# facebook/winterfell

Measured on NVIDIA H100. Metric: prover_ms, lower is better.
Workload: dtype u64

## Files before the change

include/winterfell_b200.h:

```cpp
#ifndef WINTERFELL_B200_H
#define WINTERFELL_B200_H

#include <stddef.h>
#include <stdint.h>

#ifdef __cplusplus
extern "C" {
#endif

#define WF_OK 0
#define WF_ERR_CUDA (-1)
#define WF_ERR_INVALID (-2)
#define WF_ERR_UNSUPPORTED (-3)
#define WF_ERR_STATE (-4)

#define WF_HASH_BLAKE3_256 0
#define WF_HASH_RP64_256 1
#define WF_HASH_RPJIVE64_256 2
#define WF_HASH_SHA3_256 4
#define WF_HASH_BLAKE3_192 3

typedef struct wf_ctx wf_ctx;
typedef struct wf_mat wf_mat;
typedef struct wf_tree wf_tree;
typedef struct wf_fri wf_fri;

int wf_ctx_create(wf_ctx** out, int device, void* stream);
void wf_ctx_destroy(wf_ctx* ctx);
const char* wf_last_error(const wf_ctx* ctx);
int wf_ctx_sync(wf_ctx* ctx);
uint64_t wf_ctx_launch_count(const wf_ctx* ctx);
int wf_ctx_mem_stats(const wf_ctx* ctx, uint64_t* live_buffers, uint64_t* live_bytes, uint64_t* pooled_bytes);
const char* wf_version(void);
int wf_ctx_set_profiling(wf_ctx* ctx, int on);
int wf_ctx_stage_times(wf_ctx* ctx, char* names, size_t names_cap, float* ms, size_t* count);

int wf_mat_from_host_columns(wf_ctx* ctx, const uint64_t* const* cols, uint32_t ncols, size_t nrows,
                             int ext_degree, int mont, wf_mat** out);
int wf_mat_from_device_columns(wf_ctx* ctx, const uint64_t* d_cols, uint32_t ncols, size_t nrows, wf_mat** out);
int wf_mat_select_columns(wf_ctx* ctx, const wf_mat* m, uint32_t first, uint32_t count, wf_mat** out);
int wf_mat_free(wf_ctx* ctx, wf_mat* m);
size_t wf_mat_rows(const wf_mat* m);
uint32_t wf_mat_cols(const wf_mat* m);
int wf_mat_to_columns(wf_ctx* ctx, const wf_mat* m, uint64_t* dst, int to_host, int mont);
int wf_mat_to_rows(wf_ctx* ctx, const wf_mat* m, uint64_t* dst, int to_host, int mont);
int wf_mat_read_rows(wf_ctx* ctx, const wf_mat* m, const uint64_t* positions, size_t k, uint64_t* dst, int mont);

int wf_mat_interpolate(wf_ctx* ctx, const wf_mat* evals, wf_mat** polys);
int wf_mat_evaluate(wf_ctx* ctx, const wf_mat* polys, wf_mat** evals);
int wf_mat_lde(wf_ctx* ctx, const wf_mat* polys, uint32_t log_blowup, wf_mat** lde);
int wf_mat_lde_into(wf_ctx* ctx, const wf_mat* polys, uint32_t log_blowup, wf_mat* lde);
int wf_mat_wrap_device(wf_ctx* ctx, uint64_t* d_segments, size_t rows, uint32_t cols, wf_mat** out);
int wf_trace_lde_from_host(wf_ctx* ctx, const uint64_t* const* cols, uint32_t ncols, size_t nrows, int mont, uint32_t log_blowup,
                           wf_mat** polys, wf_mat** lde);
int wf_mat_interpolate_with_offset(wf_ctx* ctx, const wf_mat* evals, uint64_t domain_offset, wf_mat** polys);

int wf_commit_rows(wf_ctx* ctx, int hash_id, const wf_mat* m, wf_tree** out);
int wf_commit_rows_partitioned(wf_ctx* ctx, int hash_id, const wf_mat* m, uint32_t partition_size, wf_tree** out);
int wf_tree_from_leaves(wf_ctx* ctx, int hash_id, const uint8_t* leaves, size_t nleaves, int leaves_on_device,
                        wf_tree** out);
int wf_tree_free(wf_ctx* ctx, wf_tree* t);
int wf_tree_root(wf_ctx* ctx, const wf_tree* t, uint8_t root[32]);
size_t wf_tree_num_leaves(const wf_tree* t);
int wf_tree_to_host(wf_ctx* ctx, const wf_tree* t, uint8_t* leaves, uint8_t* nodes);
int wf_tree_open_many(wf_ctx* ctx, const wf_tree* t, const uint64_t* positions, size_t k, uint8_t* leaves_out,
                      uint8_t* proof, size_t* proof_len);

typedef void (*wf_fri_commit_fn)(void* user, const uint8_t root[32]);
typedef void (*wf_fri_draw_fn)(void* user, uint64_t* alpha_out);
int wf_fri_build_layers(wf_ctx* ctx, int hash_id, const wf_mat* evals, int ext_degree, uint32_t folding_factor,
                        uint32_t remainder_max_degree, uint32_t blowup, wf_fri_commit_fn commit,
                        wf_fri_draw_fn draw_alpha, void* user, wf_fri** out);
int wf_fri_build_layers_default_channel(wf_ctx* ctx, int hash_id, const wf_mat* evals, int ext_degree,
                                        uint32_t folding_factor, uint32_t remainder_max_degree, uint32_t blowup,
                                        uint8_t* roots_out, size_t roots_cap, wf_fri** out);
uint32_t wf_fri_num_layers(const wf_fri* f);
size_t wf_fri_remainder(const wf_fri* f, uint64_t* coeffs, size_t cap_words);
int wf_fri_build_proof(wf_ctx* ctx, wf_fri* f, const uint64_t* positions, size_t k, uint8_t* out, size_t* len);
int wf_fri_free(wf_ctx* ctx, wf_fri* f);

int wf_prove_fib(wf_ctx* ctx, const uint64_t* const* trace_cols, int mont, uint32_t k, uint32_t log_n,
                 const uint64_t* results, const uint32_t* opts, uint8_t* proof, size_t* proof_len);

int wf_prove_air(wf_ctx* ctx, const uint64_t* air_desc, size_t air_desc_len, const uint64_t* const* trace_cols, int mont,
                 uint32_t log_n, const uint32_t* opts, uint8_t* proof, size_t* proof_len);

typedef int (*wf_aux_builder_fn)(void* user, const uint64_t* rand_elements, uint64_t* aux_out);
int wf_prove_air_aux(wf_ctx* ctx, const uint64_t* air_desc, size_t air_desc_len, const uint64_t* const* trace_cols, int mont,
                     uint32_t log_n, const uint32_t* opts, wf_aux_builder_fn aux_builder, void* aux_user, uint8_t* proof,
                     size_t* proof_len);

typedef int (*wf_aux_assertions_fn)(void* user, const uint64_t* rand_elements, uint64_t* values);
int wf_prove_air_aux_dyn(wf_ctx* ctx, const uint64_t* air_desc, size_t air_desc_len, const uint64_t* const* trace_cols, int mont,
                         uint32_t log_n, const uint32_t* opts, wf_aux_builder_fn aux_builder, wf_aux_assertions_fn aux_assertions,
                         void* aux_user, uint8_t* proof, size_t* proof_len);

int wf_prove_fib_dev(wf_ctx* ctx, const uint64_t* d_trace, uint32_t k, uint32_t log_n, const uint64_t* results,
                     const uint32_t* opts, uint8_t* proof, size_t* proof_len);

int wf_aux_build_check(const uint64_t* air_desc, size_t air_desc_len, const uint64_t* aux_build, size_t aux_build_len, uint32_t log_n,
                       char* msg, size_t msg_cap);
int wf_aux_build(wf_ctx* ctx, const uint64_t* air_desc, size_t air_desc_len, const uint64_t* aux_build, size_t aux_build_len,
                 const wf_mat* main_evals, const uint64_t* rand, uint32_t ext, wf_mat** aux);
int wf_prove_air_aux_built(wf_ctx* ctx, const uint64_t* air_desc, size_t air_desc_len, const uint64_t* aux_build, size_t aux_build_len,
                           const uint64_t* const* trace_cols, const uint64_t* d_trace, int mont, uint32_t log_n, const uint32_t* opts,
                           wf_aux_assertions_fn aux_assertions, void* aux_user, uint8_t* proof, size_t* proof_len);

int wf_prove_air_batch(wf_ctx* ctx, uint32_t batch, const uint64_t* const* air_descs, const size_t* air_desc_lens,
                       const uint64_t* aux_build, size_t aux_build_len, const uint64_t* const* trace_cols, const uint64_t* d_traces,
                       int mont, uint32_t log_n, const uint32_t* opts, uint8_t* const* proofs, size_t* proof_lens);
int wf_air_batch_check(uint32_t batch, const uint64_t* const* air_descs, const size_t* air_desc_lens, uint32_t log_n, uint32_t blowup,
                       char* msg, size_t msg_cap);

#define WF_VERIFY_ACCEPT               0
#define WF_VERIFY_MALFORMED            1
#define WF_VERIFY_OOD                  2
#define WF_VERIFY_POW                  3
#define WF_VERIFY_TRACE_QUERY          4
#define WF_VERIFY_CONSTRAINT_QUERY     5
#define WF_VERIFY_FRI_LAYER            6
#define WF_VERIFY_FRI_FOLD             7
#define WF_VERIFY_FRI_REMAINDER        8
#define WF_VERIFY_CONTEXT              9
#define WF_VERIFY_UNACCEPTABLE_OPTIONS 10
typedef int (*wf_aux_assertions_batch_fn)(void* user, uint32_t proof, const uint64_t* rand_elements, uint64_t* values);
int wf_verify_air_batch(wf_ctx* ctx, uint32_t batch, const uint64_t* const* air_descs, const size_t* air_desc_lens,
                        const uint8_t* const* proofs, const size_t* proof_lens, int hash_id,
                        const uint32_t* acceptable_opts, uint32_t num_acceptable,
                        wf_aux_assertions_batch_fn aux_assertions, void* aux_user, uint32_t* verdicts);

#define WF_VALID 0
#define WF_VIOLATION_MAIN_ASSERTION 1
#define WF_VIOLATION_AUX_ASSERTION 2
#define WF_VIOLATION_MAIN_TRANSITION 3
#define WF_VIOLATION_AUX_TRANSITION 4
#define WF_VIOLATION_DEGREES 5
#define WF_VIOLATION_CE_DOMAIN 6
typedef struct wf_validation {
    uint32_t kind;
    uint32_t index;
    uint64_t step;
    uint32_t column;
    uint32_t num_transition_constraints;
} wf_validation;
int wf_trace_validate(wf_ctx* ctx, const uint64_t* air_desc, size_t air_desc_len, const uint64_t* aux_build, size_t aux_build_len,
                      const uint64_t* const* aux_cols, const uint64_t* const* trace_cols, const uint64_t* d_trace, int mont,
                      const uint64_t* rand, uint32_t log_n, uint32_t ext, int check_degrees, wf_validation* report,
                      uint64_t* first_failing_step, uint64_t* expected_degrees, uint64_t* actual_degrees, char* msg, size_t msg_cap);
int wf_ctx_set_validation(wf_ctx* ctx, int on);

int wf_eval_constraints(wf_ctx* ctx, const uint64_t* air_desc, size_t air_desc_len, uint32_t log_n, uint32_t blowup, uint32_t ext,
                        const wf_mat* main_lde, const wf_mat* aux_lde, const uint64_t* coeffs, const uint64_t* aux_rand,
                        wf_mat** out);
int wf_composition_commit(wf_ctx* ctx, int hash_id, const wf_mat* comp_trace, uint32_t log_n, uint32_t blowup, uint32_t ext,
                          uint32_t num_cols, wf_mat** polys, wf_mat** lde, wf_tree** tree);
int wf_composition_commit_partitioned(wf_ctx* ctx, int hash_id, const wf_mat* comp_trace, uint32_t log_n, uint32_t blowup,
                                      uint32_t ext, uint32_t num_cols, uint32_t partition_size, wf_mat** polys, wf_mat** lde,
                                      wf_tree** tree);
int wf_mat_evaluate_at(wf_ctx* ctx, const wf_mat* polys, uint32_t ext, uint32_t col_ext, const uint64_t* z0, const uint64_t* z1,
                       uint64_t* out0, uint64_t* out1);
int wf_deep_compose(wf_ctx* ctx, uint32_t ext, const wf_mat* main_lde, const wf_mat* aux_lde, const wf_mat* cons_lde, uint32_t log_n,
                    const uint64_t* z, const uint64_t* coeffs, const uint64_t* ood_cur, const uint64_t* ood_next, wf_mat** out);
int wf_deep_compose_polys(wf_ctx* ctx, uint32_t ext, const wf_mat* main_polys, const wf_mat* aux_polys, const wf_mat* cons_polys,
                          uint32_t log_blowup, const uint64_t* z, const uint64_t* coeffs, wf_mat** out);

int wf_grind(wf_ctx* ctx, int hash_id, const uint8_t seed[32], uint32_t grinding, uint64_t* nonce);

typedef struct wf_comm {
    void* user;
    int rank, world;
    int (*exchange)(void* user, size_t nsend, const int* send_peer, const void* const* send, size_t nrecv,
                    const int* recv_peer, void* const* recv, size_t bytes);
    int (*all_gather_host)(void* user, const void* send, void* recv, size_t bytes);
    int (*all_reduce_sum)(void* user, void* d_buf, size_t words);
    int (*fork)(void* user);
    int (*join)(void* user);
} wf_comm;
int wf_shard_columns(uint32_t width, uint32_t world, uint32_t rank, uint32_t* first, uint32_t* count);
int wf_prove_fib_sharded(wf_ctx* ctx, const wf_comm* comm, const uint64_t* const* local_cols, const uint64_t* d_local, int mont,
                         uint32_t k, uint32_t log_n, const uint64_t* results, const uint32_t* opts, uint8_t* proof,
                         size_t* proof_len, double* stats);
int wf_prove_air_sharded(wf_ctx* ctx, const wf_comm* comm, const uint64_t* air_desc, size_t air_desc_len, const uint64_t* aux_build,
                         size_t aux_build_len, wf_aux_assertions_fn aux_assertions, void* aux_user, const uint64_t* const* local_cols,
                         const uint64_t* d_local, uint32_t local_count, int mont, uint32_t log_n, const uint32_t* opts, uint8_t* proof,
                         size_t* proof_len, double* stats);
int wf_trace_validate_sharded(wf_ctx* ctx, const wf_comm* comm, const uint64_t* air_desc, size_t air_desc_len,
                              const uint64_t* aux_build, size_t aux_build_len, const uint64_t* const* aux_cols,
                              const uint64_t* const* local_cols, const uint64_t* d_local, uint32_t local_count, int mont,
                              const uint64_t* rand, uint32_t log_n, uint32_t ext, int check_degrees, wf_validation* report,
                              uint64_t* first_failing_step, uint64_t* expected_degrees, uint64_t* actual_degrees,
                              char* msg, size_t msg_cap);

int wf_ctx_set_jit(wf_ctx* ctx, int on);
int wf_ctx_jit_stats(wf_ctx* ctx, uint64_t* compiled, uint64_t* cache_hits, uint64_t* fallbacks);
int wf_jit_compile_air(const uint64_t* air_desc, size_t air_desc_len, uint32_t ext, size_t* cubin_bytes, char* log, size_t log_cap);
int wf_air_check(const uint64_t* air_desc, size_t air_desc_len, uint32_t log_n, uint32_t blowup, char* msg, size_t msg_cap);

int wf_ntt_dev(wf_ctx* ctx, uint64_t* d_data, uint32_t log_n, uint32_t cols, int inverse);
int wf_hash_rows_dev(wf_ctx* ctx, int hash_id, const uint64_t* d_rows, size_t nrows, uint32_t cols, uint8_t* d_digests);
int wf_merkle_dev(wf_ctx* ctx, int hash_id, const uint8_t* d_leaves, size_t nleaves, uint8_t* d_nodes);
int wf_fri_fold_dev(wf_ctx* ctx, const uint64_t* d_evals, size_t len, int ext_degree, uint32_t folding_factor,
                    const uint64_t* alpha, uint64_t* d_next);

// ... 39 lines not shown
```

winterfell_b200/__init__.py:

```python
import ctypes as C
import os

import numpy as np

_HERE = os.path.dirname(os.path.abspath(__file__))
LIB_PATH = os.environ.get("WF_LIB_PATH") or os.path.join(_HERE, "libwinterfell_b200.so")

P = 0xFFFFFFFF00000001
HASH_BLAKE3_256 = 0
HASH_RP64_256 = 1
HASH_RPJIVE64_256 = 2
HASH_BLAKE3_192 = 3
HASH_SHA3_256 = 4

WF_OK = 0

u64p = C.POINTER(C.c_uint64)
u8p = C.POINTER(C.c_uint8)
vp = C.c_void_p

FRI_COMMIT_FN = C.CFUNCTYPE(None, C.c_void_p, u8p)
FRI_DRAW_FN = C.CFUNCTYPE(None, C.c_void_p, u64p)
AUX_BUILDER = C.CFUNCTYPE(C.c_int, C.c_void_p, u64p, u64p)
AUX_ASSERTIONS_BATCH = C.CFUNCTYPE(C.c_int, C.c_void_p, C.c_uint32, u64p, u64p)

VERIFY_ACCEPT, VERIFY_MALFORMED, VERIFY_OOD, VERIFY_POW, VERIFY_TRACE_QUERY, VERIFY_CONSTRAINT_QUERY, VERIFY_FRI_LAYER, \
    VERIFY_FRI_FOLD, VERIFY_FRI_REMAINDER, VERIFY_CONTEXT, VERIFY_UNACCEPTABLE_OPTIONS = range(11)

VALID, VIOLATION_MAIN_ASSERTION, VIOLATION_AUX_ASSERTION, VIOLATION_MAIN_TRANSITION, VIOLATION_AUX_TRANSITION, VIOLATION_DEGREES, \
    VIOLATION_CE_DOMAIN = range(7)


class Validation(C.Structure):
    _fields_ = [("kind", C.c_uint32), ("index", C.c_uint32), ("step", C.c_uint64), ("column", C.c_uint32),
                ("num_transition_constraints", C.c_uint32)]


def validation_dict(rep, first, exp, act, msg, check_degrees):
    k = rep.num_transition_constraints
    return {"kind": rep.kind, "index": rep.index, "step": rep.step, "column": rep.column,
            "first_failing_step": [None if int(v) == 2**64 - 1 else int(v) for v in first[:k]],
            "expected_degrees": [int(v) for v in exp[:k]] if check_degrees else None,
            "actual_degrees": [int(v) for v in act[:k]] if check_degrees else None,
            "msg": msg.value.decode(errors="replace")}


_lib = None

_SIGS = [
    ("wf_ctx_create", C.c_int, [C.POINTER(vp), C.c_int, vp]),
    ("wf_ctx_destroy", None, [vp]),
    ("wf_last_error", C.c_char_p, [vp]),
    ("wf_ctx_sync", C.c_int, [vp]),
    ("wf_ctx_launch_count", C.c_uint64, [vp]),
    ("wf_ctx_mem_stats", C.c_int, [vp, C.POINTER(C.c_uint64), C.POINTER(C.c_uint64), C.POINTER(C.c_uint64)]),
    ("wf_version", C.c_char_p, []),
    ("wf_ctx_set_profiling", C.c_int, [vp, C.c_int]),
    ("wf_ctx_stage_times", C.c_int, [vp, C.c_char_p, C.c_size_t, C.POINTER(C.c_float), C.POINTER(C.c_size_t)]),
    ("wf_mat_from_host_columns", C.c_int, [vp, C.POINTER(u64p), C.c_uint32, C.c_size_t, C.c_int, C.c_int, C.POINTER(vp)]),
    ("wf_mat_from_device_columns", C.c_int, [vp, vp, C.c_uint32, C.c_size_t, C.POINTER(vp)]),
    ("wf_mat_select_columns", C.c_int, [vp, vp, C.c_uint32, C.c_uint32, C.POINTER(vp)]),
    ("wf_mat_free", C.c_int, [vp, vp]),
    ("wf_mat_rows", C.c_size_t, [vp]),
    ("wf_mat_cols", C.c_uint32, [vp]),
    ("wf_mat_to_columns", C.c_int, [vp, vp, vp, C.c_int, C.c_int]),
    ("wf_mat_to_rows", C.c_int, [vp, vp, vp, C.c_int, C.c_int]),
    ("wf_mat_read_rows", C.c_int, [vp, vp, u64p, C.c_size_t, u64p, C.c_int]),
    ("wf_mat_interpolate", C.c_int, [vp, vp, C.POINTER(vp)]),
    ("wf_mat_evaluate", C.c_int, [vp, vp, C.POINTER(vp)]),
    ("wf_mat_lde", C.c_int, [vp, vp, C.c_uint32, C.POINTER(vp)]),
    ("wf_mat_lde_into", C.c_int, [vp, vp, C.c_uint32, vp]),
    ("wf_mat_wrap_device", C.c_int, [vp, vp, C.c_size_t, C.c_uint32, C.POINTER(vp)]),
    ("wf_trace_lde_from_host", C.c_int, [vp, C.POINTER(u64p), C.c_uint32, C.c_size_t, C.c_int, C.c_uint32, C.POINTER(vp), C.POINTER(vp)]),
    ("wf_mat_interpolate_with_offset", C.c_int, [vp, vp, C.c_uint64, C.POINTER(vp)]),
    ("wf_commit_rows", C.c_int, [vp, C.c_int, vp, C.POINTER(vp)]),
    ("wf_commit_rows_partitioned", C.c_int, [vp, C.c_int, vp, C.c_uint32, C.POINTER(vp)]),
    ("wf_tree_from_leaves", C.c_int, [vp, C.c_int, vp, C.c_size_t, C.c_int, C.POINTER(vp)]),
    ("wf_tree_free", C.c_int, [vp, vp]),
    ("wf_tree_root", C.c_int, [vp, vp, u8p]),
    ("wf_tree_num_leaves", C.c_size_t, [vp]),
    ("wf_tree_to_host", C.c_int, [vp, vp, u8p, u8p]),
    ("wf_tree_open_many", C.c_int, [vp, vp, u64p, C.c_size_t, u8p, u8p, C.POINTER(C.c_size_t)]),
    ("wf_fri_build_layers", C.c_int, [vp, C.c_int, vp, C.c_int, C.c_uint32, C.c_uint32, C.c_uint32, FRI_COMMIT_FN, FRI_DRAW_FN, vp, C.POINTER(vp)]),
    ("wf_fri_build_layers_default_channel", C.c_int, [vp, C.c_int, vp, C.c_int, C.c_uint32, C.c_uint32, C.c_uint32, u8p, C.c_size_t, C.POINTER(vp)]),
    ("wf_fri_num_layers", C.c_uint32, [vp]),
    ("wf_fri_remainder", C.c_size_t, [vp, u64p, C.c_size_t]),
    ("wf_fri_build_proof", C.c_int, [vp, vp, u64p, C.c_size_t, u8p, C.POINTER(C.c_size_t)]),
    ("wf_fri_free", C.c_int, [vp, vp]),
    ("wf_prove_fib", C.c_int, [vp, C.POINTER(u64p), C.c_int, C.c_uint32, C.c_uint32, u64p, C.POINTER(C.c_uint32), u8p, C.POINTER(C.c_size_t)]),
    ("wf_prove_air", C.c_int, [vp, u64p, C.c_size_t, C.POINTER(u64p), C.c_int, C.c_uint32, C.POINTER(C.c_uint32), u8p, C.POINTER(C.c_size_t)]),
    ("wf_prove_air_aux", C.c_int, [vp, u64p, C.c_size_t, C.POINTER(u64p), C.c_int, C.c_uint32, C.POINTER(C.c_uint32), AUX_BUILDER, vp,
                                   u8p, C.POINTER(C.c_size_t)]),
        ("wf_prove_air_aux_dyn", C.c_int, [vp, u64p, C.c_size_t, C.POINTER(u64p), C.c_int, C.c_uint32, C.POINTER(C.c_uint32), AUX_BUILDER, AUX_BUILDER, vp,
                                   u8p, C.POINTER(C.c_size_t)]),
    ("wf_aux_build_check", C.c_int, [u64p, C.c_size_t, u64p, C.c_size_t, C.c_uint32, C.c_char_p, C.c_size_t]),
    ("wf_aux_build", C.c_int, [vp, u64p, C.c_size_t, u64p, C.c_size_t, vp, u64p, C.c_uint32, C.POINTER(vp)]),
    ("wf_prove_air_aux_built", C.c_int, [vp, u64p, C.c_size_t, u64p, C.c_size_t, C.POINTER(u64p), vp, C.c_int, C.c_uint32,
                                         C.POINTER(C.c_uint32), AUX_BUILDER, vp, u8p, C.POINTER(C.c_size_t)]),
    ("wf_eval_constraints", C.c_int, [vp, u64p, C.c_size_t, C.c_uint32, C.c_uint32, C.c_uint32, vp, vp, u64p, u64p, C.POINTER(vp)]),
    ("wf_composition_commit", C.c_int, [vp, C.c_int, vp, C.c_uint32, C.c_uint32, C.c_uint32, C.c_uint32, C.POINTER(vp), C.POINTER(vp), C.POINTER(vp)]),
    ("wf_composition_commit_partitioned", C.c_int, [vp, C.c_int, vp, C.c_uint32, C.c_uint32, C.c_uint32, C.c_uint32, C.c_uint32, C.POINTER(vp),
                                                    C.POINTER(vp), C.POINTER(vp)]),
    ("wf_mat_evaluate_at", C.c_int, [vp, vp, C.c_uint32, C.c_uint32, u64p, u64p, u64p, u64p]),
    ("wf_deep_compose", C.c_int, [vp, C.c_uint32, vp, vp, vp, C.c_uint32, u64p, u64p, u64p, u64p, C.POINTER(vp)]),
    ("wf_deep_compose_polys", C.c_int, [vp, C.c_uint32, vp, vp, vp, C.c_uint32, u64p, u64p, C.POINTER(vp)]),
    ("wf_prove_fib_dev", C.c_int, [vp, vp, C.c_uint32, C.c_uint32, u64p, C.POINTER(C.c_uint32), u8p, C.POINTER(C.c_size_t)]),
    ("wf_grind", C.c_int, [vp, C.c_int, u8p, C.c_uint32, C.POINTER(C.c_uint64)]),
    ("wf_ntt_dev", C.c_int, [vp, vp, C.c_uint32, C.c_uint32, C.c_int]),
    ("wf_hash_rows_dev", C.c_int, [vp, C.c_int, vp, C.c_size_t, C.c_uint32, vp]),
    ("wf_merkle_dev", C.c_int, [vp, C.c_int, vp, C.c_size_t, vp]),
    ("wf_fri_fold_dev", C.c_int, [vp, vp, C.c_size_t, C.c_int, C.c_uint32, u64p, vp]),
    ("wf_field_ops_dev", C.c_int, [vp, vp, vp, C.c_size_t, vp]),
    ("wf_field_shifts_dev", C.c_int, [vp, vp, C.c_size_t, vp]),
    ("wf_rescue_ops_dev", C.c_int, [vp, vp, vp, C.c_size_t, vp]),
    ("wf_rescue_permute_dev", C.c_int, [vp, C.c_int, vp, vp, C.c_size_t, vp]),
    ("wf_ext_ops_dev", C.c_int, [vp, C.c_uint32, vp, vp, C.c_size_t, vp]),
    ("wf_acc_ops_dev", C.c_int, [vp, vp, vp, C.c_uint32, C.c_size_t, vp]),
    ("wf_eval_constraints_window", C.c_int, [vp, u64p, C.c_size_t, C.c_uint32, C.c_uint32, C.c_uint32, vp, vp, u64p, u64p, C.c_size_t,
                                             C.c_size_t, C.POINTER(vp)]),
    ("wf_eval_constraints_fib", C.c_int, [vp, C.c_uint32, u64p, C.c_uint32, C.c_uint32, C.c_uint32, vp, u64p, C.c_size_t, C.c_size_t,
                                          C.POINTER(vp)]),
    ("wf_eval_constraints_subcoset", C.c_int, [vp, u64p, C.c_size_t, C.c_uint32, C.c_uint32, C.c_uint32, vp, vp, u64p, u64p, C.c_size_t,
                                               C.POINTER(vp)]),
    ("wf_eval_constraints_fib_subcoset", C.c_int, [vp, C.c_uint32, u64p, C.c_uint32, C.c_uint32, C.c_uint32, vp, u64p, C.c_size_t,
                                                   C.POINTER(vp)]),
    ("wf_ctx_set_jit", C.c_int, [vp, C.c_int]),
    ("wf_ctx_jit_stats", C.c_int, [vp, C.POINTER(C.c_uint64), C.POINTER(C.c_uint64), C.POINTER(C.c_uint64)]),
    ("wf_jit_compile_air", C.c_int, [u64p, C.c_size_t, C.c_uint32, C.POINTER(C.c_size_t), C.c_char_p, C.c_size_t]),
    ("wf_air_check", C.c_int, [u64p, C.c_size_t, C.c_uint32, C.c_uint32, C.c_char_p, C.c_size_t]),
    ("wf_prove_air_batch", C.c_int, [vp, C.c_uint32, C.POINTER(u64p), C.POINTER(C.c_size_t), u64p, C.c_size_t, C.POINTER(u64p), vp, C.c_int,
                                     C.c_uint32, C.POINTER(C.c_uint32), C.POINTER(u8p), C.POINTER(C.c_size_t)]),
    ("wf_trace_validate", C.c_int, [vp, u64p, C.c_size_t, u64p, C.c_size_t, C.POINTER(u64p), C.POINTER(u64p), vp, C.c_int, u64p, C.c_uint32,
                                    C.c_uint32, C.c_int, C.POINTER(Validation), u64p, u64p, u64p, C.c_char_p, C.c_size_t]),
    ("wf_ctx_set_validation", C.c_int, [vp, C.c_int]),
    ("wf_air_batch_check", C.c_int, [C.c_uint32, C.POINTER(u64p), C.POINTER(C.c_size_t), C.c_uint32, C.c_uint32, C.c_char_p, C.c_size_t]),
    ("wf_verify_air_batch", C.c_int, [vp, C.c_uint32, C.POINTER(u64p), C.POINTER(C.c_size_t), C.POINTER(u8p), C.POINTER(C.c_size_t), C.c_int,
                                      C.POINTER(C.c_uint32), C.c_uint32, AUX_ASSERTIONS_BATCH, vp, C.POINTER(C.c_uint32)]),
    ("wf_host_hash_elements", C.c_int, [C.c_int, u64p, C.c_size_t, u8p]),
    ("wf_host_merge", C.c_int, [C.c_int, u8p, u8p]),
    ("wf_host_merge_with_int", C.c_int, [C.c_int, u8p, C.c_uint64, u8p]),
    ("wf_host_mul", C.c_uint64, [C.c_uint64, C.c_uint64]),
    ("wf_host_mul_2exp", C.c_uint64, [C.c_uint64, C.c_uint32]),
    ("wf_host_mont_to_canonical", C.c_uint64, [C.c_uint64]),
    ("wf_host_canonical_to_mont", C.c_uint64, [C.c_uint64]),
    ("wf_host_write_usize", C.c_size_t, [C.c_uint64, u8p]),
    ("wf_host_coin_draw", C.c_int, [C.c_int, u64p, C.c_size_t, u8p, C.c_int, C.c_size_t, u64p]),
    ("wf_host_build_fib_trace", C.c_int, [C.c_uint32, C.c_size_t, u64p, u64p]),
    ("wf_host_sharded_opening_plan", C.c_long, [C.c_size_t, C.c_int, C.c_int, u64p, C.c_size_t, u64p, u64p, C.c_size_t]),
    ("wf_prove_fib_sharded", C.c_int, [vp, vp, C.POINTER(u64p), vp, C.c_int, C.c_uint32, C.c_uint32, u64p, C.POINTER(C.c_uint32), u8p,
                                       C.POINTER(C.c_size_t), C.POINTER(C.c_double)]),
    ("wf_shard_columns", C.c_int, [C.c_uint32, C.c_uint32, C.c_uint32, C.POINTER(C.c_uint32), C.POINTER(C.c_uint32)]),
    ("wf_prove_air_sharded", C.c_int, [vp, vp, u64p, C.c_size_t, u64p, C.c_size_t, AUX_BUILDER, vp, C.POINTER(u64p), vp, C.c_uint32,
                                       C.c_int, C.c_uint32, C.POINTER(C.c_uint32), u8p, C.POINTER(C.c_size_t), C.POINTER(C.c_double)]),
    ("wf_trace_validate_sharded", C.c_int, [vp, vp, u64p, C.c_size_t, u64p, C.c_size_t, C.POINTER(u64p), C.POINTER(u64p), vp, C.c_uint32,
                                            C.c_int, u64p, C.c_uint32, C.c_uint32, C.c_int, C.POINTER(Validation), u64p, u64p, u64p,
                                            C.c_char_p, C.c_size_t]),
]


def declared_symbols():
    return [s[0] for s in _SIGS]


def lib():
    global _lib
    if _lib is None:
        if not os.path.exists(LIB_PATH):
            raise RuntimeError(
                f"{LIB_PATH} is missing: build it with winterfell_b200/build.sh "
                "(python -c 'import __graft_entry__ as g; g.build()'). There is no CPU fallback.")
        L = C.CDLL(LIB_PATH)
        for name, res, args in _SIGS:
            fn = getattr(L, name)
            fn.restype = res
            fn.argtypes = args
        _lib = L
    return _lib


class WfError(RuntimeError):
    pass


def _u64(a):
    a = np.ascontiguousarray(a, dtype=np.uint64)
    return a, a.ctypes.data_as(u64p)


def _u8(a):
    a = np.ascontiguousarray(a, dtype=np.uint8)
    return a, a.ctypes.data_as(u8p)


class Context:

    def __init__(self, device=0, stream=0):
        self.L = lib()
        h = vp()
        r = self.L.wf_ctx_create(C.byref(h), device, vp(stream))
        if r != WF_OK:
            raise WfError(f"wf_ctx_create failed ({r}): no usable CUDA device — this library has no CPU path")
        self.h = h

    def close(self):
        if getattr(self, "h", None):
            self.L.wf_ctx_destroy(self.h)
            self.h = None

    def __del__(self):
        try:
            self.close()
        except Exception:
            pass

    def check(self, r):
        if r != WF_OK:
            raise WfError(f"error {r}: {self.L.wf_last_error(self.h).decode()}")

    def sync(self):
        self.check(self.L.wf_ctx_sync(self.h))

    @property
    def launches(self):
        return self.L.wf_ctx_launch_count(self.h)
# ... 337 lines not shown
        ptrs, dev = None, None
        if isinstance(trace, int):
            if n is None:
                raise ValueError("n is required with a device trace pointer")
            dev = vp(trace)
        else:
            a = np.ascontiguousarray(trace, dtype=np.uint64)
            c, n = a.shape
            ptrs = (u64p * c)(*[a[j].ctypes.data_as(u64p) for j in range(c)])
        rp = aps = bp = None
        bl = 0
        if rand is not None:
            r_, rp = _u64(np.asarray(rand, dtype=np.uint64).reshape(-1))
        if aux is not None:
            x_ = np.ascontiguousarray(aux, dtype=np.uint64)
            aps = (u64p * x_.shape[0])(*[x_[j].ctypes.data_as(u64p) for j in range(x_.shape[0])])
        if aux_build is not None:
            b_, bp = _u64(aux_build)
            bl = b_.size
        cap = 1 + len(desc)
        first, exp, act = (np.zeros(cap, dtype=np.uint64) for _ in range(3))
        rep = Validation()
        msg = C.create_string_buffer(1 << 16)
        self.check(self.L.wf_trace_validate(self.h, dp, d_.size, bp, bl, aps, ptrs, dev, int(mont), rp, int(n).bit_length() - 1, ext,
                                            int(check_degrees), C.byref(rep), first.ctypes.data_as(u64p), exp.ctypes.data_as(u64p),
                                            act.ctypes.data_as(u64p), msg, 1 << 16))
        return validation_dict(rep, first, exp, act, msg, check_degrees)

    def set_validation(self, on):
        self.check(self.L.wf_ctx_set_validation(self.h, int(on)))

    def prove_fib_dev(self, d_trace, k, log_n, results, opts, out_buf=None):
        r_, rp = _u64(results)
        o_ = np.ascontiguousarray(opts, dtype=np.uint32)
        buf = out_buf if out_buf is not None else np.zeros(1 << 23, dtype=np.uint8)
        ln = C.c_size_t(buf.size)
        self.check(self.L.wf_prove_fib_dev(self.h, vp(d_trace), k, log_n, rp, o_.ctypes.data_as(C.POINTER(C.c_uint32)),
                                           buf.ctypes.data_as(u8p), C.byref(ln)))
        return buf[: ln.value].tobytes()

    def set_profiling(self, on):
        self.check(self.L.wf_ctx_set_profiling(self.h, int(on)))

    def stage_times(self):
        names = C.create_string_buffer(4096)
        ms = (C.c_float * 64)()
        cnt = C.c_size_t(64)
        self.check(self.L.wf_ctx_stage_times(self.h, names, 4096, ms, C.byref(cnt)))
        nm = [x for x in names.value.decode().split(",") if x]
        return [(nm[i], float(ms[i])) for i in range(cnt.value)]

    def grind(self, hash_id, seed: bytes, grinding):
        t_, tp = _u8(np.frombuffer(seed, dtype=np.uint8))
        nonce = C.c_uint64(0)
        self.check(self.L.wf_grind(self.h, hash_id, tp, grinding, C.byref(nonce)))
        return nonce.value

    def ntt_dev(self, dptr, log_n, cols, inverse=False):
        self.check(self.L.wf_ntt_dev(self.h, vp(dptr), log_n, cols, int(inverse)))

    def hash_rows_dev(self, hash_id, d_rows, nrows, cols, d_digests):
        self.check(self.L.wf_hash_rows_dev(self.h, hash_id, vp(d_rows), nrows, cols, vp(d_digests)))

    def merkle_dev(self, hash_id, d_leaves, nleaves, d_nodes):
        self.check(self.L.wf_merkle_dev(self.h, hash_id, vp(d_leaves), nleaves, vp(d_nodes)))

    def field_ops_dev(self, d_a, d_b, n, d_out):
        self.check(self.L.wf_field_ops_dev(self.h, vp(d_a), vp(d_b), n, vp(d_out)))

    def field_shifts_dev(self, d_a, n, d_out):
        self.check(self.L.wf_field_shifts_dev(self.h, vp(d_a), n, vp(d_out)))

    def rescue_ops_dev(self, d_a, d_b, n, d_out):
        self.check(self.L.wf_rescue_ops_dev(self.h, vp(d_a), vp(d_b), n, vp(d_out)))

    def rescue_permute_dev(self, hash_id, d_states, d_values, n, d_out):
        self.check(self.L.wf_rescue_permute_dev(self.h, hash_id, vp(d_states), vp(d_values), n, vp(d_out)))

    def set_jit(self, on):
        self.check(self.L.wf_ctx_set_jit(self.h, int(on)))

    def jit_stats(self):
        a, b, c = C.c_uint64(0), C.c_uint64(0), C.c_uint64(0)
        self.check(self.L.wf_ctx_jit_stats(self.h, C.byref(a), C.byref(b), C.byref(c)))
        return {"compiled": a.value, "cache_hits": b.value, "fallbacks": c.value}

    def ext_ops_dev(self, ext, d_a, d_b, n, d_out):
        self.check(self.L.wf_ext_ops_dev(self.h, ext, vp(d_a), vp(d_b), n, vp(d_out)))

    def acc_ops_dev(self, d_x, d_y, k, n, d_out):
        self.check(self.L.wf_acc_ops_dev(self.h, vp(d_x), vp(d_y), k, n, vp(d_out)))

    def fri_fold_dev(self, d_evals, length, ext_degree, folding, alpha, d_next):
        a_, ap = _u64(alpha)
        self.check(self.L.wf_fri_fold_dev(self.h, vp(d_evals), length, ext_degree, folding, ap, vp(d_next)))


class Mat:
    def __init__(self, ctx, h):
        self.ctx, self.h = ctx, h

    def free(self):
        if self.h:
            self.ctx.L.wf_mat_free(self.ctx.h, self.h)
            self.h = None

    @property
    def rows(self):
        return self.ctx.L.wf_mat_rows(self.h)

    @property
    def cols(self):
        return self.ctx.L.wf_mat_cols(self.h)

    def to_columns(self, mont=False):
        o = np.zeros((self.cols, self.rows), dtype=np.uint64)
        self.ctx.check(self.ctx.L.wf_mat_to_columns(self.ctx.h, self.h, vp(o.ctypes.data), 1, int(mont)))
        return o

    def to_rows(self, mont=False):
        o = np.zeros((self.rows, self.cols), dtype=np.uint64)
        self.ctx.check(self.ctx.L.wf_mat_to_rows(self.ctx.h, self.h, vp(o.ctypes.data), 1, int(mont)))
        return o

    def to_device_rows(self, dptr):
        self.ctx.check(self.ctx.L.wf_mat_to_rows(self.ctx.h, self.h, vp(dptr), 0, 0))

    def read_rows(self, positions, mont=False):
        p_, pp = _u64(positions)
        o = np.zeros((p_.size, self.cols), dtype=np.uint64)
        self.ctx.check(self.ctx.L.wf_mat_read_rows(self.ctx.h, self.h, pp, p_.size, o.ctypes.data_as(u64p), int(mont)))
        return o

    def _unary(self, fn, *extra):
        h = vp()
        self.ctx.check(fn(self.ctx.h, self.h, *extra, C.byref(h)))
        return Mat(self.ctx, h)

    def select_columns(self, first, count):
        return self._unary(self.ctx.L.wf_mat_select_columns, first, count)

    def interpolate(self):
        return self._unary(self.ctx.L.wf_mat_interpolate)

    def evaluate(self):
        return self._unary(self.ctx.L.wf_mat_evaluate)

    def lde_into(self, log_blowup, out):
        self.ctx.check(self.ctx.L.wf_mat_lde_into(self.ctx.h, self.h, log_blowup, out.h))

    def lde(self, log_blowup):
        return self._unary(self.ctx.L.wf_mat_lde, log_blowup)

    def interpolate_with_offset(self, offset):
        return self._unary(self.ctx.L.wf_mat_interpolate_with_offset, offset)


class Tree:
    def __init__(self, ctx, h):
        self.ctx, self.h = ctx, h

    def free(self):
        if self.h:
            self.ctx.L.wf_tree_free(self.ctx.h, self.h)
            self.h = None

    @property
    def num_leaves(self):
        return self.ctx.L.wf_tree_num_leaves(self.h)

    def root(self):
        o = np.zeros(32, dtype=np.uint8)
        self.ctx.check(self.ctx.L.wf_tree_root(self.ctx.h, self.h, o.ctypes.data_as(u8p)))
        return o.tobytes()

    def to_host(self):
        n = self.num_leaves
        lv = np.zeros((n, 32), dtype=np.uint8)
        nd = np.zeros((n, 32), dtype=np.uint8)
        self.ctx.check(self.ctx.L.wf_tree_to_host(self.ctx.h, self.h, lv.ctypes.data_as(u8p), nd.ctypes.data_as(u8p)))
        return lv, nd

    def open_many(self, positions):
        p_, pp = _u64(positions)
        k = p_.size
        lv = np.zeros((k, 32), dtype=np.uint8)
        cap = 64 + k * 40 * 33
        buf = np.zeros(cap, dtype=np.uint8)
        ln = C.c_size_t(cap)
        self.ctx.check(self.ctx.L.wf_tree_open_many(self.ctx.h, self.h, pp, k, lv.ctypes.data_as(u8p),
                                                    buf.ctypes.data_as(u8p), C.byref(ln)))
        return lv, buf[: ln.value].tobytes()


class Fri:
    def __init__(self, ctx, h, d):
        self.ctx, self.h, self.d = ctx, h, d

    def free(self):
        if self.h:
            self.ctx.L.wf_fri_free(self.ctx.h, self.h)
            self.h = None

    @property
    def num_layers(self):
        return self.ctx.L.wf_fri_num_layers(self.h)

    def remainder(self):
        buf = np.zeros(4096, dtype=np.uint64)
        n = self.ctx.L.wf_fri_remainder(self.h, buf.ctypes.data_as(u64p), buf.size)
        return buf[: n * self.d].copy()

    def build_proof(self, positions):
        p_, pp = _u64(positions)
        cap = 1 << 22
        buf = np.zeros(cap, dtype=np.uint8)
        ln = C.c_size_t(cap)
        self.ctx.check(self.ctx.L.wf_fri_build_proof(self.ctx.h, self.h, pp, p_.size, buf.ctypes.data_as(u8p), C.byref(ln)))
        return buf[: ln.value].tobytes()


def build_fib_trace(k, n, out=None):
    tr = out if out is not None else np.empty((2 * k, n), dtype=np.uint64)
    assert tr.shape == (2 * k, n) and tr.dtype == np.uint64 and tr.flags["C_CONTIGUOUS"]
    res = np.zeros(k, dtype=np.uint64)
    if lib().wf_host_build_fib_trace(k, n, tr.ctypes.data_as(u64p), res.ctypes.data_as(u64p)) != WF_OK:
        raise WfError("wf_host_build_fib_trace: bad arguments")
    return tr, res


def sharded_opening_plan(n_global, world, rank, positions):
    p_, pp = _u64(positions)
    cap = 64 * max(len(p_), 1) * 64
    want, idx = np.zeros(cap, dtype=np.uint64), np.zeros(cap, dtype=np.uint64)
    cnt = lib().wf_host_sharded_opening_plan(n_global, world, rank, pp, len(p_), want.ctypes.data_as(u64p), idx.ctypes.data_as(u64p), cap)
    if cnt < 0:
        raise WfError("wf_host_sharded_opening_plan: bad arguments")
    return want[:cnt].copy(), idx[:cnt].copy()


def host_hash_elements(hash_id, elems):
    e_, ep = _u64(np.asarray(elems, dtype=np.uint64).reshape(-1))
    o = np.zeros(32, dtype=np.uint8)
    lib().wf_host_hash_elements(hash_id, ep, e_.size, o.ctypes.data_as(u8p))
    return o.tobytes()


def host_merge(hash_id, a, b):
    t_, tp = _u8(np.frombuffer(a + b, dtype=np.uint8))
    o = np.zeros(32, dtype=np.uint8)
    lib().wf_host_merge(hash_id, tp, o.ctypes.data_as(u8p))
    return o.tobytes()


def host_merge_with_int(hash_id, seed, value):
    t_, tp = _u8(np.frombuffer(seed, dtype=np.uint8))
    o = np.zeros(32, dtype=np.uint8)
    lib().wf_host_merge_with_int(hash_id, tp, value, o.ctypes.data_as(u8p))
    return o.tobytes()


def air_check(desc, log_n, blowup):
    d_, dp = _u64(desc)
    msg = C.create_string_buffer(512)
    rc = lib().wf_air_check(dp, d_.size, log_n, blowup, msg, 512)
    return rc, msg.value.decode(errors="replace")


def _aux_value_count(desc):
    d = [int(x) for x in desc]
    p = 1
    def skip_degrees(p):
        cnt = d[p]; p += 1
        for _ in range(cnt):
            p += 2 + d[p + 1]
        return p
    p = skip_degrees(p)
    cnt = d[p]; p += 1
    for _ in range(cnt):
        p += 1 + d[p]
    p += 1 + d[p]
    p += 1
    p += 1 + 4 * d[p]
    cnt = d[p]; p += 1
    for _ in range(cnt):
        p += 4 + d[p + 3]
    p += 1 + d[p]
    p += 1
    if p == len(d):
        return 0
    p += 2
    p = skip_degrees(p)
    p += 1
    p += 1 + 4 * d[p]
    cnt = d[p]; p += 1
    total = 0
    for _ in range(cnt):
        total += d[p + 3]
        p += 4 + 3 * d[p + 3]
    return total


def air_batch_check(descs, log_n, blowup):
    ds = [np.ascontiguousarray(d, dtype=np.uint64) for d in descs]
    dps = (u64p * len(ds))(*[d.ctypes.data_as(u64p) for d in ds])
    dls = (C.c_size_t * len(ds))(*[d.size for d in ds])
# ... 20 lines not shown
```

winterfell_b200/csrc/capi.cu:

```cuda
#include <cuda_runtime.h>
#include <stdarg.h>
#include <stdio.h>

#include <algorithm>
#include <map>
#include <set>
#include <string>
#include <thread>
#include <utility>
#include <vector>

#include "internal.hpp"
#include "alg_hash.cuh"

void wf_mark(wf_ctx* ctx, const char* name) {
    if (!ctx->profiling) return;
    cudaEvent_t e;
    if (cudaEventCreate(&e) != cudaSuccess) return;
    cudaEventRecord(e, ctx->st);
    ctx->marks.push_back({name, e});
}
int wf_fail(wf_ctx* ctx, int code, const char* fmt, ...) {
    char buf[512];
    va_list ap;
// ... 146 lines not shown
        u64 sk = gl_mul(GL_GENERATOR, gl_pow(g, k));
        bases[k] = logR == 0 ? sk : gl_pow(sk, C);
    }
    LdeTables t{nullptr, nullptr};
    void *p, *pb;
    CK(cudaMalloc(&p, b * cnt * 8));
    CK(cudaMalloc(&pb, b * 8));
    CK(cudaMemcpyAsync(pb, bases.data(), b * 8, cudaMemcpyHostToDevice, ctx->st));
    pow_table2_kernel<<<(unsigned)((b * cnt + 255) / 256), 256, 0, ctx->st>>>((u64*)p, (u64*)pb, cnt, b);
    ctx->launches++;
    CK(cudaGetLastError());
    CK(cudaStreamSynchronize(ctx->st));
    cudaFree(pb);
    t.pre = (u64*)p;
    if (logR != 0) {
        void* q;
        CK(cudaMalloc(&q, C * 8));
        pow_table_kernel<<<(unsigned)((C + 255) / 256), 256, 0, ctx->st>>>((u64*)q, GL_GENERATOR, 1, C);
        ctx->launches++;
        CK(cudaGetLastError());
        t.pow7 = (u64*)q;
    }
    ctx->lde_tabs[key] = t;
    *out = t;
    return WF_OK;
}

static void pass_defaults(NttPassParams& p, const SegMatrix& in, const SegMatrix& out) {
    memset(&p, 0, sizeof(p));
    p.in = in.base;
    p.out = out.base;
    p.in_seg_stride = in.seg_stride;
    p.out_seg_stride = out.seg_stride;
    p.W = in.W;
    p.out_W = (u32)out.W;
    p.out_row_mul = 1;
    p.cconst = 1;
}
static int split3(wf_ctx* ctx, u32 log_n, u32* lr, u32* lc, u32* lr2, u32* lc2) {
    *lr = (log_n + 2) / 3;
    *lc = log_n - *lr;
    split_log(*lc, lr2, lc2);
    if (*lr2 == 0 || *lc2 > NTT_MAX_LOGS || *lr > NTT_MAX_LOGS)
        return wf_fail(ctx, WF_ERR_UNSUPPORTED, "transform of 2^%u points exceeds the three-pass limit", log_n);
    return WF_OK;
}

static int run_ntt(wf_ctx* ctx, const SegMatrix& in, SegMatrix& out, const SegMatrix* tmp, u32 log_n, int inverse) {
    u32 logR, logC;
    split_log(log_n, &logR, &logC);
    u64 inv_n = gl_inv(((u64)1 << log_n) % GL_P);
    NttPassParams p;
    if (logC > NTT_MAX_LOGS) {
        if (!tmp) return wf_fail(ctx, WF_ERR_STATE, "run_ntt: scratch matrix required");
        u32 lr, lc, lr2, lc2;
        CKI(split3(ctx, log_n, &lr, &lc, &lr2, &lc2));
        pass_defaults(p, in, *tmp);
        p.logS = (int)lr; p.logR = lr; p.logC = lc; p.inverse = inverse;
        p.has_post = 1; p.logM = log_n; p.a_mul = 1; p.b_mul = 0; p.cconst = inverse ? inv_n : 1;
        CKI(launch_pass(ctx, NTT_STRIDED, p, in.nseg(), 1));
        pass_defaults(p, *tmp, *tmp);
        p.in_batch_stride = p.out_batch_stride = ((size_t)1 << lc) * in.W;
        p.logS = (int)lr2; p.logR = lr2; p.logC = lc2; p.inverse = inverse;
        p.has_post = 1; p.logM = lc; p.a_mul = 1; p.b_mul = 0;
        CKI(launch_pass(ctx, NTT_STRIDED, p, in.nseg(), 1u << lr));
        pass_defaults(p, *tmp, out);
        p.in_batch_stride = ((size_t)1 << lc) * in.W;
        p.logS = (int)lc2; p.logR = lr2; p.logC = lc2; p.inverse = inverse;
        p.out_row_mul = 1u << lr; p.out_row_add = 1;
        CKI(launch_pass(ctx, NTT_CONTIG, p, in.nseg(), 1u << lr));
        return WF_OK;
    }
    if (logR == 0) {
        pass_defaults(p, in, out);
        p.logS = (int)logC; p.logR = 0; p.logC = logC; p.inverse = inverse;
        if (inverse) p.cconst = inv_n;
        return launch_pass(ctx, NTT_CONTIG, p, in.nseg(), 1);
    }
    if (!tmp) return wf_fail(ctx, WF_ERR_STATE, "run_ntt: scratch matrix required");
    pass_defaults(p, in, *tmp);
    p.logS = (int)logR; p.logR = logR; p.logC = logC; p.inverse = inverse;
    p.has_post = 1; p.logM = log_n; p.a_mul = 1; p.b_mul = 0; p.cconst = inverse ? inv_n : 1;
    CKI(launch_pass(ctx, NTT_STRIDED, p, in.nseg(), 1));
    pass_defaults(p, *tmp, out);
    p.logS = (int)logC; p.logR = logR; p.logC = logC; p.inverse = inverse;
    return launch_pass(ctx, NTT_CONTIG, p, in.nseg(), 1);
}

static int run_lde(wf_ctx* ctx, const SegMatrix& polys, SegMatrix& out, u32 log_n, u32 log_b, u32 out_col0 = 0, u32 k0 = 0, u32 k1 = 0,
                   u32 row_mul = 0, u32 row_add = 1) {
    u32 logR, logC;
    split_log(log_n, &logR, &logC);
    u32 b = 1u << log_b;
    if (k1 == 0) k1 = b;
    if (row_mul == 0) { row_mul = b; row_add = 1; }
    LdeTables tabs;
    NttPassParams p;
    if (logC > NTT_MAX_LOGS) {
        u32 lr, lc, lr2, lc2;
        CKI(split3(ctx, log_n, &lr, &lc, &lr2, &lc2));
        CKI(get_lde_tables(ctx, log_n, log_b, lr, &tabs));
        SegMatrix y = polys;
        void* yp;
        CKI(wf_dev_alloc(ctx, polys.words() * 8, &yp));
        y.base = (u64*)yp;
        int rc = WF_OK;
        for (u32 k = k0; k < k1 && rc == WF_OK; k++) {
            pass_defaults(p, polys, y);
            p.logS = (int)lr; p.logR = lr; p.logC = lc;
            p.pre_tab = tabs.pre + ((size_t)k << lr); p.pre_batch_stride = 0;
            p.has_post = 1; p.logM = log_n + log_b; p.a_mul = b; p.b_mul = 1; p.batch0 = k;
            p.ctab = tabs.pow7;
            rc = launch_pass(ctx, NTT_STRIDED, p, polys.nseg(), 1);
            if (rc != WF_OK) break;
            pass_defaults(p, y, y);
            p.in_batch_stride = p.out_batch_stride = ((size_t)1 << lc) * polys.W;
            p.logS = (int)lr2; p.logR = lr2; p.logC = lc2;
            p.has_post = 1; p.logM = lc; p.a_mul = 1; p.b_mul = 0;
            rc = launch_pass(ctx, NTT_STRIDED, p, polys.nseg(), 1u << lr);
            if (rc != WF_OK) break;
            pass_defaults(p, y, out);
            p.in_batch_stride = ((size_t)1 << lc) * polys.W;
            p.logS = (int)lc2; p.logR = lr2; p.logC = lc2;
            p.out_row_mul = row_mul << lr; p.out_row_add = row_mul; p.out_col0 = out_col0;
            p.out = out.base + (size_t)(k - k0) * row_add * out.W;
            rc = launch_pass(ctx, NTT_CONTIG, p, polys.nseg(), 1u << lr);
        }
        wf_dev_free(ctx, yp);
        return rc;
    }
    CKI(get_lde_tables(ctx, log_n, log_b, logR, &tabs));
    if (logR == 0) {
        pass_defaults(p, polys, out);
        p.logS = (int)logC; p.logR = 0; p.logC = logC;
        p.pre_tab = tabs.pre + ((size_t)k0 << log_n); p.pre_batch_stride = (size_t)1 << log_n;
        p.out_row_mul = row_mul; p.out_row_add = row_add; p.out_col0 = out_col0;
        return launch_pass(ctx, NTT_CONTIG, p, polys.nseg(), k1 - k0);
    }
    pass_defaults(p, polys, out);
    p.logS = (int)logR; p.logR = logR; p.logC = logC;
    p.pre_tab = tabs.pre + ((size_t)k0 << logR); p.pre_batch_stride = (size_t)1 << logR;
    p.has_post = 1; p.logM = log_n + log_b; p.a_mul = b; p.b_mul = 1; p.batch0 = k0;
    p.ctab = tabs.pow7;
    p.y_in_out = 1; p.out_row_mul = row_mul; p.out_row_add = row_add; p.out_col0 = out_col0;
    CKI(launch_pass(ctx, NTT_STRIDED, p, polys.nseg(), k1 - k0));
    pass_defaults(p, polys, out);
    p.in = out.base;
    p.in_seg_stride = out.seg_stride;
    p.logS = (int)logC; p.logR = logR; p.logC = logC;
    p.y_in_out = 1; p.out_row_mul = row_mul; p.out_row_add = row_add; p.out_col0 = out_col0;
    return launch_pass(ctx, NTT_CONTIG, p, polys.nseg(), k1 - k0);
}

template <int K>
__device__ __forceinline__ void field_shift_store(u64 a, u64* out, size_t n, size_t i, int slot) { out[(4 + slot) * n + i] = gl_mul_2exp<K>(a); }
__global__ void field_ops_kernel(const u64* a, const u64* b, size_t n, u64* out) {
    size_t i = (size_t)blockIdx.x * blockDim.x + threadIdx.x;
    if (i >= n) return;
    u64 x = a[i], y = b[i];
    out[i] = gl_mul(x, y);
    out[n + i] = gl_add(x, y);
    out[2 * n + i] = gl_sub(x, y);
    out[3 * n + i] = x ? gl_inv(x) : 0;
    u64 s = x, d = y;
    gl_butterfly(s, d);
    if (s != out[n + i] || d != out[2 * n + i]) out[n + i] = ~0ULL;
    field_shift_store<1>(x, out, n, i, 0);   field_shift_store<3>(x, out, n, i, 1);   field_shift_store<6>(x, out, n, i, 2);
    field_shift_store<12>(x, out, n, i, 3);  field_shift_store<24>(x, out, n, i, 4);  field_shift_store<31>(x, out, n, i, 5);
    field_shift_store<32>(x, out, n, i, 6);  field_shift_store<33>(x, out, n, i, 7);  field_shift_store<48>(x, out, n, i, 8);
    field_shift_store<63>(x, out, n, i, 9);  field_shift_store<64>(x, out, n, i, 10); field_shift_store<65>(x, out, n, i, 11);
    field_shift_store<72>(x, out, n, i, 12); field_shift_store<80>(x, out, n, i, 13); field_shift_store<84>(x, out, n, i, 14);
    field_shift_store<90>(x, out, n, i, 15); field_shift_store<95>(x, out, n, i, 16); field_shift_store<96>(x, out, n, i, 17);
}
template <int... K>
__device__ __forceinline__ void field_shifts_all(u64 x, u64* out, size_t n, size_t i, std::integer_sequence<int, K...>) {
    ((out[(size_t)K * n + i] = gl_mul_2exp<K>(x)), ...);
}
__global__ void field_shifts_kernel(const u64* a, size_t n, u64* out) {
    size_t i = (size_t)blockIdx.x * blockDim.x + threadIdx.x;
    if (i >= n) return;
    field_shifts_all(a[i], out, n, i, std::make_integer_sequence<int, 97>{});
}

__global__ void rescue_weak_kernel(const u64* a, const u64* b, size_t n, u64* out) {
    size_t i = (size_t)blockIdx.x * blockDim.x + threadIdx.x;
    if (i >= n) return;
    out[i] = gl_mul_weak(a[i], b[i]);
    out[n + i] = gl_sqr_weak(a[i]);
    out[2 * n + i] = rp64_exp7(a[i]);
}
template <int G>
__global__ void rescue_inv7_kernel(const u64* a, size_t n, u64* out) {
    size_t t = (size_t)blockIdx.x * blockDim.x + threadIdx.x;
    if (t >= n / G) return;
    u64 s[G];
#pragma unroll
    for (int e = 0; e < G; e++) s[e] = a[t * G + e];
    rp64_inv7_group<G>(s);
#pragma unroll
    for (int e = 0; e < G; e++) out[t * G + e] = s[e];
}
__global__ void rescue_mds_kernel(const u64* a, size_t n, u64* out12, u64* out8) {
    size_t t = (size_t)blockIdx.x * blockDim.x + threadIdx.x;
    if (t < n / 12) {
        u64 s[12];
        for (int e = 0; e < 12; e++) s[e] = a[t * 12 + e];
        rp64_mds(s);
        for (int e = 0; e < 12; e++) out12[t * 12 + e] = s[e];
    }
    if (t < n / 8) {
        u64 s[8];
        for (int e = 0; e < 8; e++) s[e] = a[t * 8 + e];
        rpj_mds(s);
        for (int e = 0; e < 8; e++) out8[t * 8 + e] = s[e];
    }
}
template <int HASH, int W>
__global__ void rescue_permute_kernel(const u64* in, const u64* values, size_t n, u64* out) {
    size_t i = (size_t)blockIdx.x * blockDim.x + threadIdx.x;
    if (i >= n) return;
    u64 s[W];
#pragma unroll
    for (int e = 0; e < W; e++) s[e] = in[i * W + e];
    u64 m[4], mi[4];
    alg_merge<HASH>(s, m);
    alg_merge_with_int<HASH>(s, values[i], mi);
    if (HASH == WF_HASH_RP64_256) rp64_permute(s);
    else rpj_permute(s);
#pragma unroll
    for (int e = 0; e < W; e++) out[i * W + e] = s[e];
#pragma unroll
    for (int e = 0; e < 4; e++) { out[n * W + i * 4 + e] = m[e]; out[n * (W + 4) + i * 4 + e] = mi[e]; }
}

template <int D>
__global__ void ext_ops_kernel(const u64* a, const u64* b, size_t n, u64* out) {
    size_t i = (size_t)blockIdx.x * blockDim.x + threadIdx.x;
    if (i >= n) return;
    GlExt<D> x, y;
#pragma unroll
    for (int q = 0; q < D; q++) { x.v[q] = a[i * D + q]; y.v[q] = b[i * D + q]; }
    const GlExt<D> r[6] = {ext_mul(x, y), ext_inv(x), ext_frobenius(x), ext_mul_base(x, y.v[0]), ext_add(x, y), ext_sub(x, y)};
#pragma unroll
    for (int k = 0; k < 6; k++)
#pragma unroll
        for (int q = 0; q < D; q++) out[((size_t)k * n + i) * D + q] = r[k].v[q];
}

__global__ void acc_ops_kernel(const u64* x, const u64* y, u32 k, size_t n, u64* out) {
    size_t i = (size_t)blockIdx.x * blockDim.x + threadIdx.x;
    if (i >= n) return;
    GlAcc a = acc_zero();
    for (u32 j = 0; j < k; j++) acc_mad(a, x[i * k + j], y[i * k + j]);
    u64* o = out + i * 6;
    o[0] = a.w0; o[1] = a.w1; o[2] = a.w2; o[3] = a.w3; o[4] = a.w4;
    o[5] = acc_reduce(a);
}

template <int K>
static u64 m2e(u64 x) { return gl_mul_2exp<K>(x); }

extern "C" {

const char* wf_version(void) { return "winterfell_b200 0.1 (sm_90a)"; }

int wf_ctx_create(wf_ctx** out, int device, void* stream) {
    if (!out) return WF_ERR_INVALID;
    *out = nullptr;
    int n = 0;
    cudaError_t e = cudaGetDeviceCount(&n);
    if (e != cudaSuccess || n == 0) return WF_ERR_CUDA;
    if (device < 0 || device >= n) return WF_ERR_INVALID;
    if (cudaSetDevice(device) != cudaSuccess) return WF_ERR_CUDA;
    wf_ctx* ctx = new wf_ctx();
    ctx->device = device;
    ctx->st = (cudaStream_t)stream;
    ctx->launches = 0;
    ctx->pinned = nullptr;
    ctx->pinned_bytes = 0;
    ctx->profiling = false;
    *out = ctx;
    return WF_OK;
}
void wf_ctx_destroy(wf_ctx* ctx) {
    if (!ctx) return;
    cudaSetDevice(ctx->device);
    cudaStreamSynchronize(ctx->st);
    for (auto& kv : ctx->pool) cudaFree(kv.second);
    for (auto& kv : ctx->live) cudaFree(kv.first);
    for (auto& kv : ctx->tw) cudaFree(kv.second);
    for (auto& kv : ctx->lde_tabs) { cudaFree(kv.second.pre); if (kv.second.pow7) cudaFree(kv.second.pow7); }
    if (ctx->pinned) cudaFreeHost(ctx->pinned);
    for (auto& kv : ctx->ipc_opened) cudaIpcCloseMemHandle(kv.second);
    for (auto& kv : ctx->jit_cache) if (kv.second.first) cudaLibraryUnload((cudaLibrary_t)kv.second.first);
    for (int i = 0; i < 4; i++) if (ctx->push_st[i]) { cudaStreamSynchronize(ctx->push_st[i]); cudaStreamDestroy(ctx->push_st[i]); }
    for (int i = 0; i < 16; i++) if (ctx->push_ev[i]) cudaEventDestroy(ctx->push_ev[i]);
    if (ctx->copy_st) {
        cudaStreamSynchronize(ctx->copy_st);
        for (int i = 0; i < 2; i++) { cudaEventDestroy(ctx->ev_up[i]); cudaEventDestroy(ctx->ev_used[i]); }
        cudaEventDestroy(ctx->ev_start);
        cudaStreamDestroy(ctx->copy_st);
    }
    delete ctx;
}
int wf_ctx_set_profiling(wf_ctx* ctx, int on) {
    if (!ctx) return WF_ERR_INVALID;
    ctx->profiling = on != 0;
    for (auto& m : ctx->marks) cudaEventDestroy(m.second);
    ctx->marks.clear();
    return WF_OK;
}
int wf_ctx_stage_times(wf_ctx* ctx, char* names, size_t names_cap, float* ms, size_t* count) {
    if (!ctx || !names || !ms || !count) return WF_ERR_INVALID;
    CK(cudaStreamSynchronize(ctx->st));
    size_t n = ctx->marks.size() > 0 ? ctx->marks.size() - 1 : 0, used = 0;
    if (n > *count) n = *count;
    names[0] = 0;
    for (size_t i = 0; i < n; i++) {
        CK(cudaEventElapsedTime(&ms[i], ctx->marks[i].second, ctx->marks[i + 1].second));
        const std::string& nm = ctx->marks[i + 1].first;
        if (used + nm.size() + 2 < names_cap) { memcpy(names + used, nm.c_str(), nm.size()); used += nm.size(); names[used++] = ','; names[used] = 0; }
    }
    *count = n;
    for (auto& m : ctx->marks) cudaEventDestroy(m.second);
    ctx->marks.clear();
    return WF_OK;
}
const char* wf_last_error(const wf_ctx* ctx) { return ctx ? ctx->err.c_str() : "no context (is a CUDA device present?)"; }
int wf_ctx_sync(wf_ctx* ctx) { wf_use_device(ctx); CK(cudaStreamSynchronize(ctx->st)); return WF_OK; }
uint64_t wf_ctx_launch_count(const wf_ctx* ctx) { return ctx->launches; }
int wf_ctx_mem_stats(const wf_ctx* ctx, uint64_t* live_buffers, uint64_t* live_bytes, uint64_t* pooled_bytes) {
    if (!ctx) return WF_ERR_INVALID;
    uint64_t lb = 0, pb = 0;
    for (auto& kv : ctx->live) lb += kv.second;
    for (auto& kv : ctx->pool) pb += kv.first;
    if (live_buffers) *live_buffers = ctx->live.size();
    if (live_bytes) *live_bytes = lb;
    if (pooled_bytes) *pooled_bytes = pb;
    return WF_OK;
}

int wf_mat_from_device_columns(wf_ctx* ctx, const uint64_t* d_cols, uint32_t ncols, size_t nrows, wf_mat** out) {
    if (!ctx || !d_cols || !out || ncols == 0 || nrows == 0) return wf_fail(ctx, WF_ERR_INVALID, "bad arguments");
    wf_mat* m;
    CKI(wf_mat_alloc(ctx, nrows, ncols, &m));
    CK(layout_cols_to_seg(d_cols, nrows, 1, 0, m->m, ctx->st));
    ctx->launches++;
    *out = m;
    return WF_OK;
}

int wf_mat_from_host_columns(wf_ctx* ctx, const uint64_t* const* cols, uint32_t ncols, size_t nrows, int ext_degree,
                             int mont, wf_mat** out) {
    if (!ctx || !cols || !out || ncols == 0 || nrows == 0 || ext_degree < 1 || ext_degree > 3)
        return wf_fail(ctx, WF_ERR_INVALID, "bad arguments");
    size_t col_words = nrows * ext_degree;
    void* stage;
    CKI(wf_dev_alloc(ctx, (size_t)ncols * col_words * 8, &stage));
    for (uint32_t j = 0; j < ncols; j++)
        CK(cudaMemcpyAsync((u64*)stage + (size_t)j * col_words, cols[j], col_words * 8, cudaMemcpyHostToDevice, ctx->st));
    wf_mat* m;
    int r = wf_mat_alloc(ctx, nrows, ncols * ext_degree, &m);
    if (r != WF_OK) { wf_dev_free(ctx, stage); return r; }
    CK(layout_cols_to_seg((u64*)stage, nrows, ext_degree, mont, m->m, ctx->st));
    ctx->launches++;
    wf_dev_free(ctx, stage);
    *out = m;
    return WF_OK;
}
int wf_mat_wrap_device(wf_ctx* ctx, uint64_t* d_segments, size_t rows, uint32_t cols, wf_mat** out) {
    if (!ctx || !d_segments || !out || rows == 0 || cols == 0) return wf_fail(ctx, WF_ERR_INVALID, "bad arguments");
    wf_mat* m = new wf_mat();
    m->m.rows = rows;
    m->m.cols = cols;
    m->m.W = seg_width_for(cols);
    m->m.seg_stride = rows * m->m.W;
    m->m.base = d_segments;
    *out = m;
    return WF_OK;
}
int wf_mat_select_columns(wf_ctx* ctx, const wf_mat* m, uint32_t first, uint32_t count, wf_mat** out) {
    if (!ctx || !m || !out || count == 0 || first + count > m->m.cols) return wf_fail(ctx, WF_ERR_INVALID, "bad column range");
    wf_mat* o;
    CKI(wf_mat_alloc(ctx, m->m.rows, count, &o));
    CK(layout_select_cols(m->m, first, o->m, ctx->st));
    ctx->launches++;
    *out = o;
    return WF_OK;
}
int wf_mat_free(wf_ctx* ctx, wf_mat* m) {
    if (!m) return WF_OK;
    wf_dev_free(ctx, m->m.base);
    delete m;
    return WF_OK;
}
size_t wf_mat_rows(const wf_mat* m) { return m->m.rows; }
uint32_t wf_mat_cols(const wf_mat* m) { return m->m.cols; }

static int mat_export(wf_ctx* ctx, const wf_mat* m, uint64_t* dst, int to_host, int mont, int row_major) {
    if (!ctx || !m || !dst) return wf_fail(ctx, WF_ERR_INVALID, "bad arguments");
    size_t words = m->m.rows * m->m.cols;
    u64* d = dst;
    void* tmp = nullptr;
    if (to_host) { CKI(wf_dev_alloc(ctx, words * 8, &tmp)); d = (u64*)tmp; }
    CK(layout_seg_to_flat(m->m, d, row_major, mont, ctx->st));
    ctx->launches++;
    if (to_host) {
        CK(cudaMemcpyAsync(dst, d, words * 8, cudaMemcpyDeviceToHost, ctx->st));
        CK(cudaStreamSynchronize(ctx->st));
        wf_dev_free(ctx, tmp);
    }
    return WF_OK;
}
int wf_mat_to_columns(wf_ctx* ctx, const wf_mat* m, uint64_t* dst, int to_host, int mont) { return mat_export(ctx, m, dst, to_host, mont, 0); }
int wf_mat_to_rows(wf_ctx* ctx, const wf_mat* m, uint64_t* dst, int to_host, int mont) { return mat_export(ctx, m, dst, to_host, mont, 1); }

int wf_mat_read_rows(wf_ctx* ctx, const wf_mat* m, const uint64_t* positions, size_t k, uint64_t* dst, int mont) {
    if (!ctx || !m || !positions || !dst) return wf_fail(ctx, WF_ERR_INVALID, "bad arguments");
    if (k == 0) return WF_OK;
    for (size_t i = 0; i < k; i++)
        if (positions[i] >= m->m.rows) return wf_fail(ctx, WF_ERR_INVALID, "row %llu out of range", (unsigned long long)positions[i]);
    void *dpos, *dout;
    CKI(wf_dev_alloc(ctx, k * 8, &dpos));
    CKI(wf_dev_alloc(ctx, k * m->m.cols * 8, &dout));
    CK(cudaMemcpyAsync(dpos, positions, k * 8, cudaMemcpyHostToDevice, ctx->st));
    CK(layout_gather_rows(m->m, (const u64*)dpos, k, (u64*)dout, mont, ctx->st));
    ctx->launches++;
    CK(cudaMemcpyAsync(dst, dout, k * m->m.cols * 8, cudaMemcpyDeviceToHost, ctx->st));
    CK(cudaStreamSynchronize(ctx->st));
    wf_dev_free(ctx, dpos);
    wf_dev_free(ctx, dout);
    return WF_OK;
}

static int log2_exact(size_t n, u32* out) {
    if (n == 0 || (n & (n - 1))) return -1;
    u32 l = 0;
    while (((size_t)1 << l) < n) l++;
    *out = l;
    return 0;
}

static int mat_transform(wf_ctx* ctx, const wf_mat* in, int inverse, wf_mat** out) {
    if (!ctx || !in || !out) return wf_fail(ctx, WF_ERR_INVALID, "bad arguments");
    u32 log_n;
    if (log2_exact(in->m.rows, &log_n) || log_n < 1) return wf_fail(ctx, WF_ERR_INVALID, "rows must be a power of two >= 2");
    wf_mat* o;
    CKI(wf_mat_alloc_w(ctx, in->m.rows, in->m.cols, in->m.W, &o));
    SegMatrix tmp = in->m;
    void* tp = nullptr;
    if (log_n > NTT_MAX_LOGS) {
        int r = wf_dev_alloc(ctx, in->m.words() * 8, &tp);
        if (r != WF_OK) { wf_mat_free(ctx, o); return r; }
        tmp.base = (u64*)tp;
    }
    int r = run_ntt(ctx, in->m, o->m, tp ? &tmp : nullptr, log_n, inverse);
    wf_dev_free(ctx, tp);
    if (r != WF_OK) { wf_mat_free(ctx, o); return r; }
    *out = o;
    return WF_OK;
}
int wf_mat_interpolate(wf_ctx* ctx, const wf_mat* evals, wf_mat** polys) { return mat_transform(ctx, evals, 1, polys); }
int wf_mat_evaluate(wf_ctx* ctx, const wf_mat* polys, wf_mat** evals) { return mat_transform(ctx, polys, 0, evals); }

int wf_mat_lde(wf_ctx* ctx, const wf_mat* polys, uint32_t log_blowup, wf_mat** lde) {
    if (!ctx || !polys || !lde) return wf_fail(ctx, WF_ERR_INVALID, "bad arguments");
    u32 log_n;
    if (log2_exact(polys->m.rows, &log_n) || log_n < 1) return wf_fail(ctx, WF_ERR_INVALID, "rows must be a power of two >= 2");
    if (log_blowup > 7 || log_n + log_blowup > 32) return wf_fail(ctx, WF_ERR_INVALID, "bad blowup");
    wf_mat* o;
    CKI(wf_mat_alloc(ctx, polys->m.rows << log_blowup, polys->m.cols, &o));
    int r = run_lde(ctx, polys->m, o->m, log_n, log_blowup);
    if (r != WF_OK) { wf_mat_free(ctx, o); return r; }
    *lde = o;
    return WF_OK;
}

int wf_mat_lde_into(wf_ctx* ctx, const wf_mat* polys, uint32_t log_blowup, wf_mat* lde) {
    if (!ctx || !polys || !lde) return wf_fail(ctx, WF_ERR_INVALID, "bad arguments");
    u32 log_n;
    if (log2_exact(polys->m.rows, &log_n) || log_n < 1) return wf_fail(ctx, WF_ERR_INVALID, "rows must be a power of two >= 2");
    if (log_blowup > 7 || lde->m.rows != (polys->m.rows << log_blowup) || lde->m.cols != polys->m.cols || lde->m.W != polys->m.W)
        return wf_fail(ctx, WF_ERR_INVALID, "output matrix does not match the LDE shape");
    return run_lde(ctx, polys->m, lde->m, log_n, log_blowup);
}

int wf_mat_lde_cosets(wf_ctx* ctx, const wf_mat* polys, uint32_t log_blowup, uint32_t k0, uint32_t k1, wf_mat* lde) {
    if (!ctx || !polys || !lde) return wf_fail(ctx, WF_ERR_INVALID, "bad arguments");
    u32 log_n;
    if (log2_exact(polys->m.rows, &log_n) || log_n < 1) return wf_fail(ctx, WF_ERR_INVALID, "rows must be a power of two >= 2");
    if (log_blowup > 7 || k0 >= k1 || k1 > (1u << log_blowup) || lde->m.rows != polys->m.rows * (k1 - k0) || lde->m.cols != polys->m.cols ||
        lde->m.W != polys->m.W || ((k1 - k0) & (k1 - k0 - 1)))
        return wf_fail(ctx, WF_ERR_INVALID, "coset range / output matrix do not match");
    return run_lde(ctx, polys->m, lde->m, log_n, log_blowup, 0, k0, k1, 1, (u32)polys->m.rows);
}

int wf_mat_lde_from_coset(wf_ctx* ctx, const wf_mat* polys, uint32_t log_blowup, uint32_t k0, wf_mat* lde) {
    if (!ctx || !polys || !lde) return wf_fail(ctx, WF_ERR_INVALID, "bad arguments");
    u32 log_n;
    if (log2_exact(polys->m.rows, &log_n) || log_n < 1) return wf_fail(ctx, WF_ERR_INVALID, "rows must be a power of two >= 2");
    if (log_blowup > 7 || k0 >= (1u << log_blowup) || lde->m.rows != (polys->m.rows << log_blowup) || lde->m.cols != polys->m.cols ||
        lde->m.W != polys->m.W)
        return wf_fail(ctx, WF_ERR_INVALID, "coset / output matrix do not match the LDE shape");
    SegMatrix view = lde->m;
    view.base += (size_t)k0 * view.W;
    return run_lde(ctx, polys->m, view, log_n, log_blowup, 0, k0, 1u << log_blowup);
}

int wf_trace_lde_from_host(wf_ctx* ctx, const uint64_t* const* cols, uint32_t ncols, size_t nrows, int mont, uint32_t log_blowup,
                           wf_mat** polys_out, wf_mat** lde_out) {
    return wf_trace_lde_cosetwise(ctx, cols, nullptr, ncols, nrows, mont, log_blowup, polys_out, lde_out, false, nullptr);
}
int wf_trace_lde_cosetwise(wf_ctx* ctx, const uint64_t* const* cols, const uint64_t* d_cols, uint32_t ncols, size_t nrows, int mont,
                           uint32_t log_blowup, wf_mat** polys_out, wf_mat** lde_out, bool coset_major,
                           const std::function<int(u32)>* after_coset) {
    if (!ctx || (!cols && !d_cols) || !polys_out || !lde_out || ncols == 0) return wf_fail(ctx, WF_ERR_INVALID, "bad arguments");
    u32 log_n;
    if (log2_exact(nrows, &log_n) || log_n < 1) return wf_fail(ctx, WF_ERR_INVALID, "rows must be a power of two >= 2");
    if (log_blowup > 7 || log_n + log_blowup > 32) return wf_fail(ctx, WF_ERR_INVALID, "bad blowup");
    if (coset_major && (!*lde_out || (*lde_out)->m.rows != (nrows << log_blowup) || (*lde_out)->m.W < seg_width_for(ncols) ||
                        (*lde_out)->m.cols != ncols))
        return wf_fail(ctx, WF_ERR_INVALID, "coset-major output must be preallocated");
    const int Wout = coset_major ? (*lde_out)->m.W : seg_width_for(ncols);
    const u32 nseg_out = (ncols + Wout - 1) / Wout;
    const u32 nb = 1u << log_blowup;
    auto extend = [&](const SegMatrix& pv, SegMatrix& ov, u32 out_col0, bool last) -> int {
        if (!after_coset || !last) {
            if (!coset_major) return run_lde(ctx, pv, ov, log_n, log_blowup, out_col0);
            return run_lde(ctx, pv, ov, log_n, log_blowup, out_col0, 0, nb, 1, (u32)nrows);
        }
        for (u32 k = 0; k < nb; k++) {
            SegMatrix ok = ov;
            ok.base += (coset_major ? (size_t)k * nrows : (size_t)k) * ov.W;
            if (coset_major) CKI(run_lde(ctx, pv, ok, log_n, log_blowup, out_col0, k, k + 1, 1, (u32)nrows));
            else CKI(run_lde(ctx, pv, ok, log_n, log_blowup, out_col0, k, k + 1, nb, 1));
            CKI((*after_coset)(k));
        }
        return WF_OK;
    };
    int Wc = nseg_out >= 2 ? Wout : (Wout >= 4 ? Wout / 2 : 0);
    if (d_cols || Wc == 0 || log_n < 12) {
        wf_mat* tr;
        if (d_cols) CKI(wf_mat_from_device_columns(ctx, d_cols, ncols, nrows, &tr));
        else CKI(wf_mat_from_host_columns(ctx, cols, ncols, nrows, 1, mont, &tr));
        int r = wf_mat_interpolate(ctx, tr, polys_out);
        wf_mat_free(ctx, tr);
        if (r != WF_OK) return r;
        if (!coset_major && !after_coset) return wf_mat_lde(ctx, *polys_out, log_blowup, lde_out);
        if (!coset_major) CKI(wf_mat_alloc(ctx, nrows << log_blowup, ncols, lde_out));
        const SegMatrix& pm = (*polys_out)->m;
        if (pm.W == Wout) return extend(pm, (*lde_out)->m, 0, true);
        for (u32 g = 0; g < pm.nseg(); g++) {
            SegMatrix pv = pm, ov = (*lde_out)->m;
            pv.base += (size_t)g * pm.seg_stride;
            pv.cols = std::min<u32>(pm.W, ncols - g * pm.W);
            ov.base += (size_t)(g * pm.W / Wout) * ov.seg_stride;
            ov.cols = pv.cols;
            CKI(extend(pv, ov, g * pm.W % Wout, g + 1 == pm.nseg()));
        }
        return WF_OK;
    }
    if (!ctx->copy_st) {
        CK(cudaStreamCreateWithFlags(&ctx->copy_st, cudaStreamNonBlocking));
        for (int i = 0; i < 2; i++) {
            CK(cudaEventCreateWithFlags(&ctx->ev_up[i], cudaEventDisableTiming));
            CK(cudaEventCreateWithFlags(&ctx->ev_used[i], cudaEventDisableTiming));
        }
        CK(cudaEventCreateWithFlags(&ctx->ev_start, cudaEventDisableTiming));
    }
    const u32 nchunks = (ncols + Wc - 1) / Wc;
    wf_mat *polys = nullptr, *lde = nullptr, *tr = nullptr;
    void* stage[2] = {nullptr, nullptr};
    void* tmp = nullptr;
    auto release = [&](bool results_too) {
        wf_mat_free(ctx, tr);
        for (int i = 0; i < 2; i++) wf_dev_free(ctx, stage[i]);
        wf_dev_free(ctx, tmp);
        if (results_too) { wf_mat_free(ctx, polys); if (!coset_major) wf_mat_free(ctx, lde); }
    };
    auto body = [&]() -> int {
        CKI(wf_mat_alloc_w(ctx, nrows, ncols, Wc, &polys));
        if (coset_major) lde = *lde_out;
        else CKI(wf_mat_alloc(ctx, nrows << log_blowup, ncols, &lde));
        CKI(wf_mat_alloc_w(ctx, nrows, Wc, Wc, &tr));
        for (int i = 0; i < 2; i++) CKI(wf_dev_alloc(ctx, (size_t)Wc * nrows * 8, &stage[i]));
        CKI(wf_dev_alloc(ctx, (size_t)Wc * nrows * 8, &tmp));
        if (lde->m.W > (int)ncols) CK(cudaMemsetAsync(lde->m.base, 0, lde->m.words() * 8, ctx->st));
        CK(cudaEventRecord(ctx->ev_start, ctx->st));
        CK(cudaStreamWaitEvent(ctx->copy_st, ctx->ev_start, 0));
        for (u32 k = 0; k < nchunks; k++) {
            const u32 c0 = k * Wc, cw = std::min<u32>(Wc, ncols - c0);
            const int sb = k & 1;
            if (k >= 2) CK(cudaStreamWaitEvent(ctx->copy_st, ctx->ev_used[sb], 0));
            for (u32 j = 0; j < cw; j++)
                CK(cudaMemcpyAsync((u64*)stage[sb] + (size_t)j * nrows, cols[c0 + j], nrows * 8, cudaMemcpyHostToDevice, ctx->copy_st));
            CK(cudaEventRecord(ctx->ev_up[sb], ctx->copy_st));
            CK(cudaStreamWaitEvent(ctx->st, ctx->ev_up[sb], 0));
            SegMatrix trv = tr->m;
            trv.cols = cw;
            CK(layout_cols_to_seg((const u64*)stage[sb], nrows, 1, mont, trv, ctx->st));
            CK(cudaEventRecord(ctx->ev_used[sb], ctx->st));
            ctx->launches++;
            SegMatrix pv = polys->m;
            pv.base = polys->m.base + (size_t)k * polys->m.seg_stride;
            pv.cols = cw;
            SegMatrix tv = trv;
            tv.base = (u64*)tmp;
            CKI(run_ntt(ctx, trv, pv, &tv, log_n, 1));
            SegMatrix ov = lde->m;
            ov.base = lde->m.base + (size_t)(c0 / Wout) * lde->m.seg_stride;
            ov.cols = cw;
            CKI(extend(pv, ov, c0 % Wout, k + 1 == nchunks));
        }
        return WF_OK;
    };
    int rc = body();
    if (rc != WF_OK) {
        cudaStreamSynchronize(ctx->copy_st);
        release(true);
        return rc;
    }
    release(false);
    *polys_out = polys;
    *lde_out = lde;
    return WF_OK;
}

int wf_mat_interpolate_with_offset(wf_ctx* ctx, const wf_mat* evals, uint64_t domain_offset, wf_mat** polys) {
// ... 676 lines not shown
```

winterfell_b200/csrc/internal.hpp:

```cpp
#pragma once
#include <cuda_runtime.h>

#include <algorithm>
#include <map>
#include <set>
#include <string>
#include <functional>
#include <vector>

#include "../../include/winterfell_b200.h"
#include "commit.cuh"
#include "fri.cuh"
#include "host_transcript.hpp"
#include "layout.cuh"
#include "ntt.cuh"

struct LdeTables {
    u64* pre;
    u64* pow7;
};

struct wf_ctx {
    int device;
    cudaStream_t st;
    std::string err;
    uint64_t launches;
    std::multimap<size_t, void*> pool;
    std::map<void*, size_t> live;
    std::map<u32, u64*> tw;
    std::map<u32, u64*> round_tw;
    std::map<std::pair<u32, u32>, u64*> pow_tab;
    std::map<std::pair<u32, u32>, LdeTables> lde_tabs;
    void* pinned;
    size_t pinned_bytes;
    cudaStream_t copy_st = nullptr;
    cudaEvent_t ev_up[2], ev_used[2], ev_start;
    std::map<std::string, void*> ipc_opened;
    cudaStream_t push_st[4] = {nullptr, nullptr, nullptr, nullptr};
    cudaEvent_t push_ev[16] = {};
    std::map<std::string, std::pair<void*, void*>> jit_cache;
    bool jit_enabled = true;
    bool validate = false;
    uint64_t jit_compiled = 0, jit_hits = 0, jit_fallbacks = 0;
    bool profiling;
    std::vector<std::pair<std::string, cudaEvent_t>> marks;
};
void wf_mark(wf_ctx* ctx, const char* name);

struct wf_mat {
    SegMatrix m;
};
struct wf_tree {
    int hash_id;
    size_t nleaves;
    u64* leaves;
    u64* nodes;
};

static inline u32 log2_ceil(size_t n) { return n <= 1 ? 0 : 64 - (u32)__builtin_clzll((unsigned long long)(n - 1)); }

static inline void wf_host_dft(std::vector<u64>& v, size_t n, int d, bool inverse, u64 offset) {
    const u32 log_n = log2_ceil(n);
    u64 w0 = n > 1 ? gl_root_of_unity(log_n) : 1;
    if (inverse) w0 = gl_inv(w0);
    if (!inverse && offset != 1) {
        u64 f = 1;
        for (size_t i = 0; i < n; i++) { for (int c = 0; c < d; c++) v[i * d + c] = gl_mul(v[i * d + c], f); f = gl_mul(f, offset); }
    }
    for (size_t i = 0; i < n; i++) {
        size_t j = 0;
        for (u32 b = 0; b < log_n; b++) j |= ((i >> b) & 1) << (log_n - 1 - b);
        if (j > i) for (int c = 0; c < d; c++) std::swap(v[i * d + c], v[j * d + c]);
    }
    for (size_t len = 2; len <= n; len <<= 1) {
        u64 wl = gl_pow(w0, n / len);
        for (size_t s = 0; s < n; s += len) {
            u64 w = 1;
            for (size_t i = 0; i < len / 2; i++) {
                for (int c = 0; c < d; c++) {
                    u64 a = v[(s + i) * d + c], b = gl_mul(v[(s + i + len / 2) * d + c], w);
                    v[(s + i) * d + c] = gl_add(a, b);
                    v[(s + i + len / 2) * d + c] = gl_sub(a, b);
                }
                w = gl_mul(w, wl);
            }
        }
    }
    if (inverse) {
        u64 scale = gl_inv((u64)n % GL_P), oinv = gl_inv(offset);
        for (size_t i = 0; i < n; i++) {
            for (int c = 0; c < d; c++) v[i * d + c] = gl_mul(v[i * d + c], scale);
            scale = gl_mul(scale, oinv);
        }
    }
}

int wf_fail(wf_ctx* ctx, int code, const char* fmt, ...);
int pinned_reserve(wf_ctx* ctx, size_t bytes);
std::string wf_jit_source(int D, u32 w, u32 nper, u32 nregs, const std::vector<u32>& prog, const std::vector<u64>& consts, u32 aw, u32 nr,
                          u32 naregs, const std::vector<u32>& aprog);
int wf_jit_compile(const std::string& src, std::vector<char>& cubin, std::string& log);
int wf_jit_get_kernel(wf_ctx* ctx, const std::string& src, cudaKernel_t* kernel);
int wf_dev_alloc(wf_ctx* ctx, size_t bytes, void** out);
void wf_dev_free(wf_ctx* ctx, void* p);
struct AuxBuildCol {
    u32 kind = 0;
    u64 init[3] = {0, 0, 0};
    u32 num_regs = 0;
    std::vector<u32> prog;
};
struct AuxBuildHost {
    u32 aw = 0;
    std::vector<u64> consts;
    std::vector<AuxBuildCol> cols;
};
const char* wf_aux_build_parse(const u64* d, size_t len, u32 w, u32 aw, u32 np, u32 nr, AuxBuildHost& out);
int wf_aux_build_run(wf_ctx* ctx, const AuxBuildHost& b, const wf_mat* main, u32 w, const std::vector<std::vector<u64>>& periodic,
                     const u64* rnd, u32 nr, int D, wf_mat** out);
struct DevScratch {
    wf_ctx* ctx;
    std::vector<void*> bufs;
    explicit DevScratch(wf_ctx* c) : ctx(c) {}
    DevScratch(const DevScratch&) = delete;
    DevScratch& operator=(const DevScratch&) = delete;
    ~DevScratch() { for (void* p : bufs) if (p) wf_dev_free(ctx, p); }
    int alloc(size_t bytes, void** out) {
        int r = wf_dev_alloc(ctx, bytes, out);
        if (r == WF_OK) bufs.push_back(*out);
        return r;
    }
    void forget(void* p) { for (void*& q : bufs) if (q == p) { q = nullptr; return; } }
    void free(void* p) { if (!p) return; forget(p); wf_dev_free(ctx, p); }
    void* keep(void* p) { forget(p); return p; }
};
int wf_mat_alloc(wf_ctx* ctx, size_t rows, u32 cols, wf_mat** out);
int wf_mat_alloc_w(wf_ctx* ctx, size_t rows, u32 cols, int W, wf_mat** out);
extern "C" int wf_trace_lde_cosetwise(wf_ctx* ctx, const uint64_t* const* cols, const uint64_t* d_cols, uint32_t ncols, size_t nrows, int mont,
                           uint32_t log_blowup, wf_mat** polys_out, wf_mat** lde_out, bool coset_major,
                           const std::function<int(u32)>* after_coset);
extern "C" int wf_mat_lde_cosets(wf_ctx* ctx, const wf_mat* polys, uint32_t log_blowup, uint32_t k0, uint32_t k1, wf_mat* lde);
extern "C" int wf_mat_lde_from_coset(wf_ctx* ctx, const wf_mat* polys, uint32_t log_blowup, uint32_t k0, wf_mat* lde);
struct PublicCoin;
struct Digest;
struct wf_fri;
int wf_fri_build_layers_coin(wf_ctx* ctx, int hash_id, const wf_mat* evals, int d, uint32_t folding, uint32_t rem_max_deg,
                             uint32_t blowup, PublicCoin& coin, std::vector<Digest>& commitments, wf_fri** out,
                             wf_mat* consume = nullptr);
int wf_get_twiddles(wf_ctx* ctx, u32 log_n, const u64** out);
struct wf_tree;
int wf_fri_layer_tree(wf_ctx* ctx, int hash_id, const u64* vals, size_t len, int d, int ld, int nf, wf_tree** out);
struct OpenPlan {
    u32 depth;
    u32 digest_bytes = 32;
    std::vector<u64> want;
    std::vector<std::vector<size_t>> vec_slots;
    std::vector<size_t> leaf_slot;
};
int wf_open_plan(wf_ctx* ctx, size_t n, const uint64_t* positions, size_t k, OpenPlan& pl);
void wf_open_finish(const OpenPlan& pl, const uint8_t* got, uint8_t* leaves_out, ByteVec& proof);
struct GatherBatch {
    struct RowJob { SegMatrix m; std::vector<u64> pos; size_t idx_off, out_off; };
    struct DigJob { const wf_tree* t; OpenPlan plan; std::vector<u64> idx; size_t idx_off, out_off; };
    std::vector<RowJob> rows;
    std::vector<DigJob> digs;
    const wf_comm* comm = nullptr;
    u64* result = nullptr;
    size_t add_rows(const SegMatrix& m, const std::vector<u64>& pos);
    int add_opening(wf_ctx* ctx, const wf_tree* t, const std::vector<u64>& pos, size_t* id);
    int add_opening_sharded(wf_ctx* ctx, const wf_tree* t, size_t n_global, int world, int rank, const std::vector<u64>& pos,
                            size_t* id, std::vector<std::pair<size_t, u64>>* top_slots);
    int run(wf_ctx* ctx);
    const u64* row_result(size_t id) const { return result + rows[id].out_off; }
    const u8* digest_result(size_t id) const { return (const u8*)(result + digs[id].out_off); }
    u64* digest_words(size_t id) { return result + digs[id].out_off; }
};
struct FriLayer {
    u64* evals;
    size_t len;
    wf_tree* tree;
};
struct wf_fri {
    int hash_id, d, ld;
    u32 folding, blowup;
    std::vector<FriLayer> layers;
    std::vector<u64> remainder;
};

struct FriProofPlan { std::vector<size_t> row_ids, dig_ids; std::vector<size_t> nq; };
int wf_fri_queue_proof(wf_ctx* ctx, wf_fri* f, const std::vector<u64>& positions, GatherBatch& gb, FriProofPlan& plan);
void wf_fri_finish_proof(const wf_fri* f, const GatherBatch& gb, const FriProofPlan& plan, ByteVec& out,
                         const FriProofPlan* before = nullptr);
int wf_tree_open_many_bytes(wf_ctx* ctx, const wf_tree* t, const uint64_t* positions, size_t k, uint8_t* leaves_out,
                            ByteVec& proof);

#define CK(call)                                                                                          \
    do {                                                                                                  \
        cudaError_t _e = (call);                                                                          \
        if (_e != cudaSuccess)                                                                            \
            return wf_fail(ctx, WF_ERR_CUDA, "%s:%d %s: %s", __FILE__, __LINE__, #call, cudaGetErrorString(_e)); \
    } while (0)
#define CKI(call)                   \
    do {                            \
        int _r = (call);            \
        if (_r != WF_OK) return _r; \
    } while (0)
```

winterfell_b200/csrc/ntt.cuh:

```cuda
#pragma once
#include <cuda_runtime.h>
#include <stdint.h>

#include "gl64.cuh"

#define NTT_LANES 8
#ifndef NTT_THREADS
#define NTT_THREADS 512
#endif
#ifndef NTT_LD_BATCH
#define NTT_LD_BATCH 8
#endif
#ifndef NTT_MIN_BLOCKS
#define NTT_MIN_BLOCKS 2
#endif
#define NTT_MAX_LOGS 11

struct NttPassParams {
    const u64* in;
    u64* out;
    size_t in_seg_stride, out_seg_stride;
    size_t in_batch_stride, out_batch_stride;
    int W;
    int logS;
    u32 logR, logC;
    int inverse;
    u32 out_row_mul, out_row_add;
    int y_in_out;
    u32 out_W, out_col0;
    const u64* sub_tw;
    const u64* pre_tab;
    size_t pre_batch_stride;
    int has_post;
    const u64* master;
    u32 logM;
    u32 a_mul, b_mul;
    u32 batch0;
    const u64 *tw_hi, *tw_lo;
    u32 tw_split;
    int vec_in, vec_out;
    const u64* ctab;
    u64 cconst;
};

enum { NTT_STRIDED = 0, NTT_CONTIG = 1 };

size_t ntt_pass_smem_bytes(const NttPassParams& p);
cudaError_t ntt_launch_pass(int mode, const NttPassParams& p, u32 n_segments, u32 n_batch, cudaStream_t st);
#define NTT2_MIN_LOGS 6
cudaError_t ntt2_launch_pass(int mode, const NttPassParams& p, u32 n_segments, u32 n_batch, cudaStream_t st);
size_t ntt2_tw_entries(int logS);
cudaError_t ntt2_build_tw(int logS, u64* d_out, cudaStream_t st);
```

winterfell_b200/csrc/ntt2.cu:

```cuda
#include "minidft.cuh"
#include "ntt.cuh"

#ifndef NTT2_THREADS
#define NTT2_THREADS 256
#endif
#ifndef NTT2_MINB
#define NTT2_MINB 2
#endif
#define NTT2_TILE_ELEMS 8192

template <int LOGS>
struct Plan {
    static constexpr int rounds = LOGS >= 9 ? 3 : 2;
    static constexpr int r0 = (LOGS == 8) ? 4 : 3;
    static constexpr int r1 = (LOGS == 11 || LOGS == 8 || LOGS == 7) ? 4 : 3;
    static constexpr int r2 = LOGS >= 9 ? LOGS - r0 - r1 : 0;
    static_assert(LOGS >= 6 && LOGS <= 11, "plan covers 2^6 .. 2^11");
    static_assert(r0 + r1 + r2 == LOGS && (rounds == 2 || (r2 == 3 || r2 == 4)), "radices must add up");
    static constexpr int lanes = LOGS == 11 ? 4 : 8;
    static constexpr int tw0_entries = 1 << LOGS;
    static constexpr int tw1_entries = rounds == 3 ? (1 << (LOGS - r0)) : 0;
    static constexpr int tw_entries = tw0_entries + tw1_entries;
};
template <int LOGS> __host__ __device__ constexpr int plan_radix(int k) { return k == 0 ? Plan<LOGS>::r0 : (k == 1 ? Plan<LOGS>::r1 : Plan<LOGS>::r2); }
template <int LOGS> __host__ __device__ constexpr int plan_stage(int k) { return k == 0 ? 0 : (k == 1 ? Plan<LOGS>::r0 : Plan<LOGS>::r0 + Plan<LOGS>::r1); }

template <int LK>
__host__ __device__ constexpr u32 swz_const(u32 r) {
    u32 x = r >> LK, h = 0;
    while (x) { h ^= x & ((1u << LK) - 1); x >>= LK; }
    return h;
}
template <int LK>
__host__ __device__ constexpr u32 swz_lo(u32 Q) { return swz_const<LK>(Q) ^ (Q & ((1u << LK) - 1)); }
template <int LK>
__host__ __device__ constexpr u32 swz_hi(u32 Q) { return Q & ~((1u << LK) - 1); }
__host__ __device__ constexpr u32 brev_const(u32 v, int bits) {
    u32 r = 0;
    for (int i = 0; i < bits; i++) r |= ((v >> i) & 1u) << (bits - 1 - i);
    return r;
}
template <int LOGS, int LK, u32 STEP, u32 N, u32 IT = 0, class F>
__device__ __forceinline__ void for_brev_rows(F&& f) {
    if constexpr (IT < N) {
        constexpr u32 c = brev_const(IT * STEP, LOGS);
        f(IT, swz_lo<LK>(c), swz_hi<LK>(c));
        for_brev_rows<LOGS, LK, STEP, N, IT + 1>(f);
    }
}
template <int LK>
__device__ __forceinline__ u32 swz_hash(u32 r) {
    if (LK == 1) return __popc(r >> 1) & 1;
    u32 x = r >> 2;
    x ^= x >> 4;
    x ^= x >> 8;
    x ^= x >> 2;
    return x & 3;
}
template <int LK>
__device__ __forceinline__ u32 prow(u32 r) { return r ^ swz_hash<LK>(r); }

__device__ __forceinline__ void bulk_init(u64* mbar, int tid) {
    if (tid == 0) {
        u32 mb = (u32)__cvta_generic_to_shared(mbar);
        asm volatile("mbarrier.init.shared::cta.b64 [%0], 1;" ::"r"(mb));
        asm volatile("fence.mbarrier_init.release.cluster;" ::: "memory");
    }
}
__device__ __forceinline__ void bulk_expect(u64* mbar, u32 bytes) {
    u32 mb = (u32)__cvta_generic_to_shared(mbar);
    asm volatile("mbarrier.arrive.expect_tx.shared::cta.b64 _, [%0], %1;" ::"r"(mb), "r"(bytes) : "memory");
}
__device__ __forceinline__ void bulk_copy(void* smem_dst, const void* gsrc, u32 bytes, u64* mbar) {
    u32 mb = (u32)__cvta_generic_to_shared(mbar), dst = (u32)__cvta_generic_to_shared(smem_dst);
    asm volatile("cp.async.bulk.shared::cluster.global.mbarrier::complete_tx::bytes [%0], [%1], %2, [%3];" ::"r"(dst), "l"(gsrc), "r"(bytes),
                 "r"(mb)
                 : "memory");
}
__device__ __forceinline__ void bulk_wait(u64* mbar) {
    u32 mb = (u32)__cvta_generic_to_shared(mbar), done = 0;
    while (!done)
        asm volatile("{\n\t.reg .pred p;\n\tmbarrier.try_wait.parity.shared::cta.b64 p, [%1], 0;\n\tselp.u32 %0, 1, 0, p;\n\t}" : "=r"(done) : "r"(mb) : "memory");
}

__device__ __forceinline__ void cp_async16(void* smem_dst, const void* gsrc, bool ok) {
    const u32 dst = (u32)__cvta_generic_to_shared(smem_dst);
    asm volatile("cp.async.cg.shared.global [%0], [%1], 16, %2;" ::"r"(dst), "l"(gsrc), "r"(ok ? 16 : 0) : "memory");
}
__device__ __forceinline__ void cp_async8(void* smem_dst, const void* gsrc, bool ok) {
    const u32 dst = (u32)__cvta_generic_to_shared(smem_dst);
    asm volatile("cp.async.ca.shared.global [%0], [%1], 8, %2;" ::"r"(dst), "l"(gsrc), "r"(ok ? 8 : 0) : "memory");
}
__device__ __forceinline__ void cp_async_commit() { asm volatile("cp.async.commit_group;" ::: "memory"); }
__device__ __forceinline__ void cp_async_wait_all() { asm volatile("cp.async.wait_group 0;" ::: "memory"); }

template <int LOGS, int K>
__device__ __forceinline__ void tile_round(u64* __restrict__ s, const u64* __restrict__ tw, const u64* __restrict__ pre, int tid) {
    constexpr int LANES = Plan<LOGS>::lanes, LK = LANES == 8 ? 1 : 2;
    constexpr int R = plan_radix<LOGS>(K), ST = plan_stage<LOGS>(K);
    constexpr int LOGSPAN = LOGS - ST - R;
    constexpr u32 SPAN = 1u << LOGSPAN;
    constexpr bool LAST = LOGSPAN == 0;
    constexpr u32 TASKS = (1u << LOGS) * LANES / 16;
    if (R == 4) {
#pragma unroll 1
        for (u32 task = tid; task < TASKS; task += NTT2_THREADS) {
            const u32 lane = task % LANES, bf = task / LANES;
            const u32 lo = bf & (SPAN - 1), base = ((bf >> LOGSPAN) << (LOGSPAN + 4)) + lo;
            const u32 bh = base ^ swz_hash<LK>(base);
            u64* pr[1 << LK];
#pragma unroll
            for (int v = 0; v < (1 << LK); v++) pr[v] = s + ((bh ^ v) * LANES + lane);
            u64 x[16];
#pragma unroll
            for (int q = 0; q < 16; q++) x[q] = pr[swz_lo<LK>((u32)q << LOGSPAN)][swz_hi<LK>((u32)q << LOGSPAN) * LANES];
            if (K == 0 && pre) {
#pragma unroll
                for (int q = 0; q < 16; q++) x[q] = gl_mul(x[q], __ldg(pre + base + ((u32)q << LOGSPAN)));
            }
            mini_dft<4>(x);
            if (!LAST) {
                const ulonglong2* t2 = reinterpret_cast<const ulonglong2*>(tw + (size_t)lo * 16);
#pragma unroll
                for (int h = 0; h < 8; h++) {
                    const ulonglong2 w = t2[h];
                    if (h > 0) x[2 * h] = gl_mul(x[2 * h], w.x);
                    x[2 * h + 1] = gl_mul(x[2 * h + 1], w.y);
                }
            }
#pragma unroll
            for (int q = 0; q < 16; q++) pr[swz_lo<LK>((u32)q << LOGSPAN)][swz_hi<LK>((u32)q << LOGSPAN) * LANES] = x[q];
        }
    } else {
        constexpr int LP = LANES / 2;
#pragma unroll 1
        for (u32 task = tid; task < TASKS; task += NTT2_THREADS) {
            const u32 lp = task % LP, bf = task / LP;
            const u32 lo = bf & (SPAN - 1), base = ((bf >> LOGSPAN) << (LOGSPAN + 3)) + lo;
            const u32 bh = base ^ swz_hash<LK>(base);
            ulonglong2* pr[1 << LK];
#pragma unroll
            for (int v = 0; v < (1 << LK); v++) pr[v] = reinterpret_cast<ulonglong2*>(s + ((bh ^ v) * LANES + 2 * lp));
            u64 xa[8], xb[8];
#pragma unroll
            for (int q = 0; q < 8; q++) {
                const ulonglong2 v = pr[swz_lo<LK>((u32)q << LOGSPAN)][swz_hi<LK>((u32)q << LOGSPAN) * (LANES / 2)];
                xa[q] = v.x;
                xb[q] = v.y;
            }
            if (K == 0 && pre) {
#pragma unroll
                for (int q = 0; q < 8; q++) {
                    const u64 f = __ldg(pre + base + ((u32)q << LOGSPAN));
                    xa[q] = gl_mul(xa[q], f);
                    xb[q] = gl_mul(xb[q], f);
                }
            }
            mini_dft<3>(xa);
            mini_dft<3>(xb);
            if (!LAST) {
                const ulonglong2* t2 = reinterpret_cast<const ulonglong2*>(tw + (size_t)lo * 8);
#pragma unroll
                for (int h = 0; h < 4; h++) {
                    const ulonglong2 w = t2[h];
                    if (h > 0) { xa[2 * h] = gl_mul(xa[2 * h], w.x); xb[2 * h] = gl_mul(xb[2 * h], w.x); }
                    xa[2 * h + 1] = gl_mul(xa[2 * h + 1], w.y);
                    xb[2 * h + 1] = gl_mul(xb[2 * h + 1], w.y);
                }
            }
#pragma unroll
            for (int q = 0; q < 8; q++) pr[swz_lo<LK>((u32)q << LOGSPAN)][swz_hi<LK>((u32)q << LOGSPAN) * (LANES / 2)] = make_ulonglong2(xa[q], xb[q]);
        }
    }
}

template <int MODE, int LOGS>
__global__ void __launch_bounds__(NTT2_THREADS, NTT2_MINB) ntt2_pass_kernel(const NttPassParams p) {
    extern __shared__ __align__(16) u64 smem[];
    constexpr int LANES = Plan<LOGS>::lanes, LK = LANES == 8 ? 1 : 2, LP = LANES / 2;
    constexpr u32 S = 1u << LOGS;
    const int tid = threadIdx.x;
    const int W = p.W, logW = 31 - __clz(W);
    const int T = W >= LANES ? 1 : (LANES >> logW);
    const int chunks = W >= LANES ? W / LANES : 1;
    u64* s = smem;
    u64* rtw = s + (size_t)S * LANES;
    u64* ctw = rtw + Plan<LOGS>::tw_entries;
    u64* mbar = ctw + (p.has_post ? (size_t)S * T : 0);

    const bool ymap = p.y_in_out;
    const u32 tc = ymap ? blockIdx.y : blockIdx.x;
    const u32 tile = tc / chunks, q0 = (tc % chunks) * LANES;
    const u32 g = ymap ? blockIdx.z : blockIdx.y, b = ymap ? blockIdx.x : blockIdx.z;
    const u32 R = 1u << p.logR, C = 1u << p.logC;
    const u32 ncols = MODE == NTT_STRIDED ? C : R;

    {
        const u64* in = p.in + (size_t)g * p.in_seg_stride + (size_t)b * p.in_batch_stride;
        const u32 lp = tid % LP;
        const u32 l0 = 2 * lp;
        const u32 t0 = W >= LANES ? 0 : (l0 >> logW), t1 = W >= LANES ? 0 : ((l0 + 1) >> logW);
        const u32 w0 = W >= LANES ? q0 + l0 : (l0 & (W - 1)), w1 = W >= LANES ? q0 + l0 + 1 : ((l0 + 1) & (W - 1));
        const u32 c0 = tile * T + t0, c1 = tile * T + t1;
        const bool ok0 = c0 < ncols, ok1 = c1 < ncols;
        const bool yin = MODE == NTT_CONTIG && ymap;
        const u64 istride = MODE == NTT_STRIDED ? ((u64)W << p.logC) : (yin ? ((u64)p.out_row_mul << p.logR) * p.out_W : (u64)W);
        const u64* a0 = MODE == NTT_STRIDED ? in + (size_t)c0 * W + w0
                        : yin ? in + ((size_t)c0 * p.out_row_mul + (size_t)b * p.out_row_add) * p.out_W + p.out_col0 + w0
                              : in + (((size_t)c0 << p.logC) * W + w0);
        const u64* a1 = MODE == NTT_STRIDED ? in + (size_t)c1 * W + w1
                        : yin ? in + ((size_t)c1 * p.out_row_mul + (size_t)b * p.out_row_add) * p.out_W + p.out_col0 + w1
                              : in + (((size_t)c1 << p.logC) * W + w1);
        if (!ok0) a0 = p.in;
        if (!ok1) a1 = p.in;
        const u64 s0 = ok0 ? istride : 0, s1 = ok1 ? istride : 0;
        const bool vec = p.vec_in;
        constexpr u32 ROWS_PER_IT = NTT2_THREADS / LP;
#pragma unroll 4
        for (u32 i = tid / LP; i < S; i += ROWS_PER_IT) {
            u64* dst = s + prow<LK>(i) * LANES + l0;
            if (vec) {
                cp_async16(dst, a0 + i * s0, ok0);
            } else {
                cp_async8(dst, a0 + i * s0, ok0);
                cp_async8(dst + 1, a1 + i * s1, ok1);
            }
        }
        cp_async_commit();
    }

    bulk_init(mbar, tid);
    __syncthreads();
    if (tid == 0) {
        bulk_expect(mbar, Plan<LOGS>::tw_entries * 8);
        bulk_copy(rtw, p.sub_tw, Plan<LOGS>::tw_entries * 8, mbar);
    }

    if (p.has_post && T == 1) {
        const u32 M = 1u << p.logM, lo_mask = (1u << p.tw_split) - 1, c = tile;
        auto wpow = [&](u64 e64) {
            u32 e = (u32)(e64 & (M - 1));
            if (p.inverse && e) e = M - e;
            return gl_mul(p.tw_hi[e >> p.tw_split], p.tw_lo[e & lo_mask]);
        };
        u64 K = wpow((u64)(p.batch0 + b) * p.b_mul * c);
        if (p.ctab) K = gl_mul(K, p.ctab[c < ncols ? c : 0]);
        if (p.cconst != 1) K = gl_mul(K, p.cconst);
        const u64 step = wpow((u64)NTT2_THREADS * p.a_mul * c);
        u64 x = gl_mul(K, wpow((u64)tid * p.a_mul * c));
        for (u32 j = tid; j < S; j += NTT2_THREADS) {
            ctw[j] = x;
            x = gl_mul(x, step);
        }
    } else if (p.has_post) {
        const u32 M = 1u << p.logM, lo_mask = (1u << p.tw_split) - 1;
        for (u32 idx = tid; idx < S * (u32)T; idx += NTT2_THREADS) {
            const u32 j = idx / T, tt = idx % T, c = tile * T + tt;
            u64 e64 = ((u64)j * p.a_mul + (u64)(p.batch0 + b) * p.b_mul) * c;
            u32 e = (u32)(e64 & (M - 1));
            if (p.inverse && e) e = M - e;
            u64 x = gl_mul(p.tw_hi[e >> p.tw_split], p.tw_lo[e & lo_mask]);
            if (p.ctab) x = gl_mul(x, p.ctab[c < ncols ? c : 0]);
            if (p.cconst != 1) x = gl_mul(x, p.cconst);
            ctw[idx] = x;
        }
    }

    cp_async_wait_all();
    bulk_wait(mbar);
    __syncthreads();

    tile_round<LOGS, 0>(s, rtw, p.pre_tab ? p.pre_tab + (size_t)b * p.pre_batch_stride : nullptr, tid);
    __syncthreads();
    if (Plan<LOGS>::rounds == 3) {
        tile_round<LOGS, 1>(s, rtw + Plan<LOGS>::tw0_entries, nullptr, tid);
        __syncthreads();
        tile_round<LOGS, 2>(s, nullptr, nullptr, tid);
    } else {
        tile_round<LOGS, 1>(s, nullptr, nullptr, tid);
    }
    __syncthreads();

    u64* out = p.out + (size_t)g * p.out_seg_stride + (size_t)b * p.out_batch_stride;
    {
        const u32 lp = tid % LP, l0 = 2 * lp;
        const u32 t0 = W >= LANES ? 0 : (l0 >> logW), t1 = W >= LANES ? 0 : ((l0 + 1) >> logW);
        const u32 w0 = W >= LANES ? q0 + l0 : (l0 & (W - 1)), w1 = W >= LANES ? q0 + l0 + 1 : ((l0 + 1) & (W - 1));
        const u32 c0 = tile * T + t0, c1 = tile * T + t1;
        const bool ok0 = c0 < ncols, ok1 = c1 < ncols;
        u64 *o0, *o1, jstride;
        if (MODE == NTT_STRIDED && ymap) {
            o0 = out + (((size_t)c0 << p.logR) * p.out_row_mul + (size_t)b * p.out_row_add) * p.out_W + p.out_col0 + w0;
            o1 = out + (((size_t)c1 << p.logR) * p.out_row_mul + (size_t)b * p.out_row_add) * p.out_W + p.out_col0 + w1;
            jstride = (u64)p.out_row_mul * p.out_W;
        } else if (MODE == NTT_STRIDED) {
            o0 = out + (size_t)c0 * W + w0;
            o1 = out + (size_t)c1 * W + w1;
            jstride = (u64)W << p.logC;
        } else {
            o0 = out + ((size_t)c0 * p.out_row_mul + (size_t)b * p.out_row_add) * p.out_W + p.out_col0 + w0;
            o1 = out + ((size_t)c1 * p.out_row_mul + (size_t)b * p.out_row_add) * p.out_W + p.out_col0 + w1;
            jstride = ((u64)p.out_row_mul << p.logR) * p.out_W;
        }
        const bool post = p.has_post, scale = !p.has_post && p.cconst != 1, vec = p.vec_out;
        const u32 inv_mask = p.inverse ? (S - 1) : 0;
        constexpr u32 ROWS_PER_IT = NTT2_THREADS / LP;
        if (!p.inverse && vec && T == 1) {
            const u32 j0 = tid / LP, r0 = __brev(j0) >> (32 - LOGS), rh = r0 ^ swz_hash<LK>(r0);
            const ulonglong2* pr[1 << LK];
#pragma unroll
            for (int v = 0; v < (1 << LK); v++) pr[v] = reinterpret_cast<const ulonglong2*>(s + ((rh ^ v) * LANES + l0));
            const u64* cj = ctw + j0;
            u64* oj = o0 + (u64)j0 * jstride;
            const u64 ostep = (u64)ROWS_PER_IT * jstride;
            for_brev_rows<LOGS, LK, ROWS_PER_IT, S / ROWS_PER_IT>([&](u32 it, u32 lo, u32 hi) {
                ulonglong2 v = pr[lo][hi * (LANES / 2)];
                if (post) {
                    const u64 f = cj[it * ROWS_PER_IT];
                    v.x = gl_mul(v.x, f);
                    v.y = gl_mul(v.y, f);
                } else if (scale) {
                    v.x = gl_mul(v.x, p.cconst);
                    v.y = gl_mul(v.y, p.cconst);
                }
                if (ok0) *reinterpret_cast<ulonglong2*>(oj + it * ostep) = v;
            });
            return;
// ... 92 lines not shown
```

winterfell_b200/csrc/prover.cu:

```cuda
#include <algorithm>
#include <chrono>

#include "internal.hpp"
#include "air_host.hpp"
#include "blake3.cuh"
#include "alg_hash.cuh"

#include "constraints_generic.cuh"

#ifndef FIB_ROWS_D3
#define FIB_ROWS_D3 2
#endif
struct FibEvalParams {
    SegMatrix lde;
    SegMatrix out;
    u32 k, log_n, log_blowup, log_ce_blowup;
    const u64* coef;
    u64 K0[3], K1[3];
    const u64* tw_ce;
    u64 zt[8];
    u64 last;
    size_t row0, ce_rows;
    u32 log_step;
};
// ... 1027 lines not shown
    *lde_out = clde;
    return WF_OK;
}
int composition_commit(wf_ctx* ctx, int h, const wf_mat* comp, u32 log_n, u32 log_b, int D, u32 kc, wf_mat** polys_out,
                       wf_mat** lde_out, wf_tree** tree_out, u32 partition_words = 0) {
    wf_mat *cpolys = nullptr, *clde = nullptr;
    CKI(composition_polys(ctx, comp, log_n, D, kc, &cpolys));
    int r = composition_lde(ctx, comp, cpolys, log_n, log_b, kc, &clde);
    if (r == WF_OK) {
        wf_mark(ctx, "composition_lde");
        if (tree_out) r = wf_commit_rows_partitioned(ctx, h, clde, partition_words, tree_out);
    }
    if (r != WF_OK) { wf_mat_free(ctx, cpolys); wf_mat_free(ctx, clde); return r; }
    *polys_out = cpolys;
    *lde_out = clde;
    return WF_OK;
}

template <int D>
int deep_compose(wf_ctx* ctx, const wf_mat* lde, const wf_mat* alde, const wf_mat* clde, u32 kc, u32 log_N,
                 const std::vector<GlExt<D>>& dc, const GlExt<D>& z, const GlExt<D>& zg, const GlExt<D>& Sz, const GlExt<D>& Szg,
                 wf_mat** out, size_t row0 = 0, size_t nrows = 0) {
    const u32 c = lde->m.cols, aw = alde ? alde->m.cols / D : 0, ct = c + aw;
    const size_t N = nrows ? nrows : ((size_t)1 << log_N);
    for (const GlExt<D>* w : {&z, &zg}) {
        bool base = true;
        for (int q = 1; q < D; q++) base = base && w->v[q] == 0;
        if (base && gl_sqr_n(gl_mul(w->v[0], 2635249152773512046ULL), (int)log_N) == 1)
            return wf_fail(ctx, WF_ERR_INVALID, "DEEP point %s lies on the LDE domain: its denominators vanish", w == &z ? "z" : "z*g");
    }
    DeepPoint<D> pz, pzg;
    if (!deep_point<D>(z, pz) || !deep_point<D>(zg, pzg)) return wf_fail(ctx, WF_ERR_STATE, "conjugates of the out-of-domain point are inconsistent");
    u64 *d_dt, *d_dq, *d_da;
    CKI(upload_ext<D>(ctx, dc, 0, ct + kc, &d_dt));
    d_da = d_dt + (size_t)c * D;
    d_dq = d_dt + (size_t)ct * D;
    wf_mat* deep;
    CKI(wf_mat_alloc(ctx, N, D, &deep));
    DeepParams p;
    p.trace = lde->m; p.cons = clde->m; p.out = deep->m; p.c = c; p.kc = kc; p.log_N = log_N;
    p.row0 = row0; p.nrows = nrows;
    p.tcc = d_dt; p.ccc = d_dq; p.acc = d_da; p.aw = aw;
    p.aux = aw ? alde->m : lde->m;
    CKI(wf_get_twiddles(ctx, log_N, &p.tw_N));
    const size_t coef_bytes = (size_t)(c + aw + kc) * D * 8;
    deep_sum_kernel<D><<<(unsigned)((N + DEEP_SUM_THREADS - 1) / DEEP_SUM_THREADS), DEEP_SUM_THREADS, coef_bytes, ctx->st>>>(p);
    const size_t rows_per_thread = DEEP_ROWS;
    size_t threads = (N + rows_per_thread - 1) / rows_per_thread;
    deep_div_kernel<D><<<(unsigned)((threads + 255) / 256), 256, 0, ctx->st>>>(p, pz, pzg, Sz, Szg);
    ctx->launches += 2;
    CK(cudaGetLastError());
    wf_dev_free(ctx, d_dt);
    *out = deep;
    return WF_OK;
}

template <int D>
int deep_compose_polys(wf_ctx* ctx, const wf_mat* polys, const wf_mat* apolys, const wf_mat* cpolys, u32 kc, u32 log_b,
                       const std::vector<GlExt<D>>& dc, const GlExt<D>& z, const GlExt<D>& zg, wf_mat** out) {
    const u32 c = polys->m.cols, aw = apolys ? apolys->m.cols / D : 0, ct = c + aw;
    const size_t n = polys->m.rows, ntiles = (n + SYN_TILE - 1) / SYN_TILE;
    const u32 log_n = log2_ceil(n);
    DevScratch tmp(ctx);
    u64* d_dt;
    CKI(upload_ext<D>(ctx, dc, 0, ct + kc, &d_dt));
    tmp.bufs.push_back(d_dt);
    void* d_agg;
    CKI(tmp.alloc((ntiles * (1 + SYN_WARPS + SYN_THREADS) + SYN_PW) * 2 * D * 8, &d_agg));
    SynDivBufs sb;
    sb.agg = (u64*)d_agg;
    sb.wsuf = sb.agg + ntiles * 2 * D;
    sb.tsuf = sb.wsuf + ntiles * SYN_WARPS * 2 * D;
    sb.pw = sb.tsuf + ntiles * SYN_THREADS * 2 * D;
    wf_mat* quot;
    CKI(wf_mat_alloc(ctx, n, D, &quot));
    DeepParams p{};
    p.trace = polys->m; p.cons = cpolys->m; p.out = quot->m; p.c = c; p.kc = kc; p.log_N = log_n;
    p.tcc = d_dt; p.acc = d_dt + (size_t)c * D; p.ccc = d_dt + (size_t)ct * D; p.aw = aw;
    p.aux = aw ? apolys->m : polys->m;
    deep_sum_kernel<D><<<(unsigned)((n + DEEP_SUM_THREADS - 1) / DEEP_SUM_THREADS), DEEP_SUM_THREADS, (size_t)(ct + kc) * D * 8, ctx->st>>>(p);
    SynDivParams<D> sp;
    sp.b[0] = z; sp.b[1] = zg;
    for (int pt = 0; pt < 2; pt++) {
        sp.b_items[pt] = ext_pow(sp.b[pt], SYN_ITEMS);
        sp.b_tile[pt] = ext_pow(sp.b[pt], SYN_TILE);
        sp.lvl[pt][0] = sp.b_items[pt];
        for (int k = 1; k < 8; k++) sp.lvl[pt][k] = ext_mul(sp.lvl[pt][k - 1], sp.lvl[pt][k - 1]);
    }
    syn_div_reduce<D><<<(unsigned)ntiles, SYN_THREADS, 0, ctx->st>>>(quot->m.base, n, sp, sb);
    syn_div_carry<D><<<1, SYN_THREADS, 0, ctx->st>>>(sb.agg, ntiles, sp, sb.pw);
    syn_div_apply<D><<<(unsigned)ntiles, SYN_THREADS, 0, ctx->st>>>(quot->m.base, n, sp, sb);
    ctx->launches += 4;
    const cudaError_t e = cudaGetLastError();
    const int r = e == cudaSuccess ? wf_mat_lde(ctx, quot, log_b, out) : wf_fail(ctx, WF_ERR_CUDA, "DEEP quotient launch: %s", cudaGetErrorString(e));
    wf_mat_free(ctx, quot);
    return r;
}

static int validation_result(wf_ctx* ctx, int r, const TraceReport& rep) {
    if (r != WF_OK) return r;
    return rep.kind == WF_VALID ? WF_OK : wf_fail(ctx, WF_ERR_INVALID, "%s", rep.msg.c_str());
}

struct ProofScope {
    wf_ctx* ctx;
    std::vector<wf_mat**> mats;
    std::vector<wf_tree**> trees;
    wf_fri** fri = nullptr;
    explicit ProofScope(wf_ctx* c) : ctx(c) {}
    void own(std::initializer_list<wf_mat**> l) { mats.insert(mats.end(), l); }
    void own(std::initializer_list<wf_tree**> l) { trees.insert(trees.end(), l); }
    void drop(wf_mat*& m) { wf_mat_free(ctx, m); m = nullptr; }
    ~ProofScope() {
        if (fri && *fri) wf_fri_free(ctx, *fri);
        for (wf_mat** m : mats) if (*m) wf_mat_free(ctx, *m);
        for (wf_tree** t : trees) if (*t) wf_tree_free(ctx, *t);
    }
};

template <int D>
int prove_air(wf_ctx* ctx, const AirHost& air_in, const uint64_t* const* trace_cols, const uint64_t* d_trace, int mont, u32 log_n,
              const Options& o, wf_aux_builder_fn aux_builder, void* aux_user, std::vector<u8>& proof_out,
              wf_aux_assertions_fn aux_assertions = nullptr, const AuxBuildHost* aux_build = nullptr) {
    AirHost air_dyn;
    if (aux_assertions) air_dyn = air_in;
    const AirHost& air = aux_assertions ? air_dyn : air_in;
    const int h = o.hash_id;
    const size_t n = (size_t)1 << log_n;
    const u32 log_b = log2_ceil(o.blowup);
    const size_t N = n << log_b;
    const u32 c = air.w, kc = air.num_comp_cols(n), log_ceb = air.log_ce_blowup();
    const u32 aw = air.aw;
    if (aw && !aux_builder && !aux_build) return wf_fail(ctx, WF_ERR_INVALID, "multi-segment AIR needs an aux trace builder");
    const bool validate = ctx->validate && !air.is_fib;
    if (log_ceb > log_b) return wf_fail(ctx, WF_ERR_INVALID, "blowup factor too small for the constraint degrees");
    for (auto& col : air.periodic) if (col.size() > n) return wf_fail(ctx, WF_ERR_INVALID, "periodic column longer than the trace");
    CKI(validate_degrees(ctx, air.all_degrees(), n));
    CKI(validate_assertions(ctx, air.aux_asserts, n, 3, "aux assertion"));
    CKI(validate_assertions(ctx, air.asserts, n, 1, "assertion"));
    Channel ch(h, context_seed(air, n, o));

    wf_mat *trace = nullptr, *polys = nullptr, *lde = nullptr, *atrace = nullptr, *apolys = nullptr, *alde = nullptr, *comp = nullptr,
           *cpolys = nullptr, *clde = nullptr, *deep = nullptr;
    wf_tree *ttree = nullptr, *atree = nullptr, *ctree = nullptr;
    wf_fri* fri = nullptr;
    ProofScope scope(ctx);
    scope.own({&trace, &polys, &lde, &atrace, &apolys, &alde, &comp, &cpolys, &clde, &deep});
    scope.own({&ttree, &atree, &ctree});
    scope.fri = &fri;
    wf_mark(ctx, "start");
    if (d_trace) {
        CKI(wf_mat_from_device_columns(ctx, d_trace, c, n, &trace));
        wf_mark(ctx, "trace_upload_layout");
        CKI(wf_mat_interpolate(ctx, trace, &polys));
        if (!aux_build && !validate) scope.drop(trace);
        wf_mark(ctx, "trace_interpolate");
        CKI(wf_mat_lde(ctx, polys, log_b, &lde));
    } else {
        CKI(wf_trace_lde_from_host(ctx, trace_cols, c, n, mont, log_b, &polys, &lde));
    }
    wf_mark(ctx, "trace_lde");
    CKI(wf_commit_rows_partitioned(ctx, h, lde, o.part_words(c, 1), &ttree));
    u8 root[32];
    CKI(wf_tree_root(ctx, ttree, root));
    wf_mark(ctx, "trace_commit");
    ch.commit(root);

    std::vector<u64> rnd_flat;
    if (aw) {
        for (u32 i = 0; i < air.nr; i++) { GlExt<D> e = draw_ext<D>(ch.coin); for (int q = 0; q < D; q++) rnd_flat.push_back(e.v[q]); }
        std::vector<u64> rnd_user = rnd_flat;
        if (mont) for (u64& v : rnd_user) v = gl_mul(v, 0xFFFFFFFFULL);
        std::vector<u64> aux_host;
        if (aux_build) {
            if (!trace) CKI(wf_mat_evaluate(ctx, polys, &trace));
            CKI(wf_aux_build_run(ctx, *aux_build, trace, c, air.periodic, rnd_flat.data(), air.nr, D, &atrace));
            if (!validate) scope.drop(trace);
            wf_mark(ctx, "aux_build");
        } else {
            aux_host.resize((size_t)aw * n * D);
            if (aux_builder(aux_user, rnd_user.data(), aux_host.data()) != 0) return wf_fail(ctx, WF_ERR_INVALID, "aux trace builder failed");
        }
        if (aux_assertions) {
            std::vector<u64> vals = get_aux_assertion_words(air_dyn, D, mont);
            if (aux_assertions(aux_user, rnd_user.data(), vals.data()) != 0) return wf_fail(ctx, WF_ERR_INVALID, "aux assertion callback failed");
            if (!set_aux_assertion_words(air_dyn, vals.data(), D, mont))
                return wf_fail(ctx, WF_ERR_INVALID, "aux assertion value is not a canonical field element");
        }
        if (!aux_build) {
            std::vector<const u64*> cols(aw);
            for (u32 j = 0; j < aw; j++) cols[j] = &aux_host[(size_t)j * n * D];
            CKI(wf_mat_from_host_columns(ctx, cols.data(), aw, n, D, mont, &atrace));
        }
        CKI(wf_mat_interpolate(ctx, atrace, &apolys));
        if (!validate) scope.drop(atrace);
        CKI(wf_mat_lde(ctx, apolys, log_b, &alde));
        CKI(wf_commit_rows_partitioned(ctx, h, alde, o.part_words(aw, D), &atree));
        CKI(wf_tree_root(ctx, atree, root));
        wf_mark(ctx, "aux_commit");
        ch.commit(root);
    }
    if (validate) {
        if (!trace) CKI(wf_mat_evaluate(ctx, polys, &trace));
        TraceReport rep;
        CKI(validation_result(ctx, wf_check_trace(ctx, air, trace, atrace, rnd_flat.data(), log_n, D, rep), rep));
        scope.drop(trace);
        scope.drop(atrace);
    }

    std::vector<GlExt<D>> cc = draw_coeffs<D>(ch.coin, o.batch_c, air.num_constraints());
    const size_t m = comp_subcoset_rows(n, kc);
    const u32 log_step = m < (n << log_ceb) ? log_n + log_ceb - log2_ceil(m) : 0;
    CKI(eval_constraints<D>(ctx, air, lde, alde, cc, rnd_flat, log_n, log_b, &comp, 0, 0, log_step));
    if (validate) {
        TraceReport rep;
        CKI(validation_result(ctx, wf_check_degrees(ctx, air, lde, alde, rnd_flat.data(), log_n, log_b, D, rep), rep));
    }
    wf_mark(ctx, "constraint_eval");
    CKI(composition_commit(ctx, h, comp, log_n, log_b, D, kc, &cpolys, &clde, &ctree, o.part_words(kc, D)));
    scope.drop(comp);
    CKI(wf_tree_root(ctx, ctree, root));
    wf_mark(ctx, "composition_commit");
    ch.commit(root);

    GlExt<D> z = draw_ext<D>(ch.coin);
    GlExt<D> zg = ext_mul_base(z, gl_root_of_unity(log_n));
    std::vector<std::vector<GlExt<D>>> ood;
    {
        std::vector<const wf_mat*> mats = {polys, cpolys};
        if (aw) mats.push_back(apolys);
        CKI(ood_eval<D>(ctx, mats, z, zg, ood));
    }
    std::vector<GlExt<D>>&t_cur = ood[0], &t_nxt = ood[1];
    std::vector<GlExt<D>> q_cur = ext_from_components<D>(ood[2]), q_nxt = ext_from_components<D>(ood[3]);
    if (aw) {
        auto a_cur = ext_from_components<D>(ood[4]), a_nxt = ext_from_components<D>(ood[5]);
        t_cur.insert(t_cur.end(), a_cur.begin(), a_cur.end());
        t_nxt.insert(t_nxt.end(), a_nxt.begin(), a_nxt.end());
    }
    const u32 ct = c + aw;
    ByteVec ood_t, ood_q;
    ch.coin.reseed(ood_frames<D>(h, t_cur, t_nxt, q_cur, q_nxt, &ood_t, &ood_q));
    wf_mark(ctx, "ood_frames");
    std::vector<GlExt<D>> dc = draw_coeffs<D>(ch.coin, o.batch_d, ct + kc);
    CKI(deep_compose_polys<D>(ctx, polys, apolys, cpolys, kc, log_b, dc, z, zg, &deep));
    wf_mark(ctx, "deep_composition");
    {
        std::vector<Digest> fri_roots;
        CKI(wf_fri_build_layers_coin(ctx, h, deep, D, o.folding, o.rem_max_deg, o.blowup, ch.coin, fri_roots, &fri, deep));
        for (auto& r : fri_roots) ch.commitments.bytes(r.b, WF_DIGEST_BYTES(h));
    }
    scope.drop(deep);
    wf_mark(ctx, "fri_layers");
    u64 nonce;
    CKI(grind_on_device(ctx, h, ch.coin.seed, o.grinding, &nonce));
    if (ch.coin.check_leading_zeros(nonce) < o.grinding) return wf_fail(ctx, WF_ERR_STATE, "grinding self-check failed");
    std::vector<u64> pos;
    if (!query_positions(ch.coin, o.num_queries, N, nonce, pos)) return wf_fail(ctx, WF_ERR_STATE, "failed to draw query positions");
    wf_mark(ctx, "grinding");
    ByteVec w;
    write_context(w, air, log_n, o);
    w.u8_((u8)pos.size());
    w.u16_((uint16_t)ch.commitments.v.size());
    w.bytes(ch.commitments.v.data(), ch.commitments.v.size());
    GatherBatch gb;
    FriProofPlan fplan;
    size_t tr_rows = gb.add_rows(lde->m, pos), cr_rows = gb.add_rows(clde->m, pos), tr_dig, cr_dig;
    size_t ar_rows = 0, ar_dig = 0;
    if (aw) ar_rows = gb.add_rows(alde->m, pos);
    CKI(gb.add_opening(ctx, ttree, pos, &tr_dig));
    CKI(gb.add_opening(ctx, ctree, pos, &cr_dig));
    if (aw) CKI(gb.add_opening(ctx, atree, pos, &ar_dig));
    CKI(wf_fri_queue_proof(ctx, fri, pos, gb, fplan));
    CKI(gb.run(ctx));
    write_queries(gb, tr_rows, tr_dig, pos.size() * c, w);
    if (aw) write_queries(gb, ar_rows, ar_dig, pos.size() * aw * D, w);
    write_queries(gb, cr_rows, cr_dig, pos.size() * kc * D, w);
    w.u16_((uint16_t)ood_t.v.size()); w.bytes(ood_t.v.data(), ood_t.v.size());
    w.u16_((uint16_t)ood_q.v.size()); w.bytes(ood_q.v.data(), ood_q.v.size());
    wf_fri_finish_proof(fri, gb, fplan, w);
    w.u64_(nonce);
    wf_mark(ctx, "queries_and_proof");
    proof_out.swap(w.v);
    return WF_OK;
}

__global__ void __launch_bounds__(256) coset_interleave_kernel(SegMatrix src, SegMatrix dst, size_t rows_j, u32 b) {
    const size_t idx = (size_t)blockIdx.x * blockDim.x + threadIdx.x;
    const int W = dst.W;
    if (idx >= dst.rows * (size_t)W) return;
    const size_t row = idx / W;
    const u32 w = (u32)(idx % W), g = blockIdx.y;
    const size_t j = row / b, k = row % b;
    dst.base[(size_t)g * dst.seg_stride + idx] = src.base[(size_t)g * src.seg_stride + (k * rows_j + j) * W + w];
}

struct ShardCtx {
    wf_ctx* ctx;
    const wf_comm* cm;
    int G, r;
    double bytes_sent = 0, bytes_overlapped = 0, ncoll = 0, ms_small = 0;
    bool forked = false;
    bool peer_push = false;
    int fork() {
        if (cm->fork) { if (cm->fork(cm->user) != 0) return wf_fail(ctx, WF_ERR_STATE, "fork callback failed"); forked = true; }
        return WF_OK;
    }
    int join() {
        if (forked) { forked = false; if (cm->join(cm->user) != 0) return wf_fail(ctx, WF_ERR_STATE, "join callback failed"); }
        return WF_OK;
// ... 1395 lines not shown
```

Baseline: 79.57.

## Fuse trace interpolation second pass with LDE first pass in one kernel

Adds a fused interpolate-and-extend path for 2^22-row traces with width-8 segments. It runs the strided inverse pass, then one kernel that finishes the inverse NTT tile, writes the coefficients, and reuses them in registers to run the first forward pass for every coset. A final contiguous pass completes the LDE. The aim is to skip a full global-memory round trip of the polynomial matrix and some launches, at the cost of a temporary buffer and a path that only applies to one specific shape.

```diff
diff --git a/include/winterfell_b200.h b/include/winterfell_b200.h
--- a/include/winterfell_b200.h
+++ b/include/winterfell_b200.h
@@ -49,6 +49,7 @@
 int wf_mat_interpolate(wf_ctx* ctx, const wf_mat* evals, wf_mat** polys);
 int wf_mat_evaluate(wf_ctx* ctx, const wf_mat* polys, wf_mat** evals);
 int wf_mat_lde(wf_ctx* ctx, const wf_mat* polys, uint32_t log_blowup, wf_mat** lde);
+int wf_mat_interpolate_lde(wf_ctx* ctx, const wf_mat* evals, uint32_t log_blowup, wf_mat** polys, wf_mat** lde);
 int wf_mat_lde_into(wf_ctx* ctx, const wf_mat* polys, uint32_t log_blowup, wf_mat* lde);
 int wf_mat_wrap_device(wf_ctx* ctx, uint64_t* d_segments, size_t rows, uint32_t cols, wf_mat** out);
 int wf_trace_lde_from_host(wf_ctx* ctx, const uint64_t* const* cols, uint32_t ncols, size_t nrows, int mont, uint32_t log_blowup,
diff --git a/winterfell_b200/__init__.py b/winterfell_b200/__init__.py
--- a/winterfell_b200/__init__.py
+++ b/winterfell_b200/__init__.py
@@ -70,6 +70,7 @@
     ("wf_mat_evaluate", C.c_int, [vp, vp, C.POINTER(vp)]),
     ("wf_mat_lde", C.c_int, [vp, vp, C.c_uint32, C.POINTER(vp)]),
     ("wf_mat_lde_into", C.c_int, [vp, vp, C.c_uint32, vp]),
+    ("wf_mat_interpolate_lde", C.c_int, [vp, vp, C.c_uint32, C.POINTER(vp), C.POINTER(vp)]),
     ("wf_mat_wrap_device", C.c_int, [vp, vp, C.c_size_t, C.c_uint32, C.POINTER(vp)]),
     ("wf_trace_lde_from_host", C.c_int, [vp, C.POINTER(u64p), C.c_uint32, C.c_size_t, C.c_int, C.c_uint32, C.POINTER(vp), C.POINTER(vp)]),
     ("wf_mat_interpolate_with_offset", C.c_int, [vp, vp, C.c_uint64, C.POINTER(vp)]),
@@ -713,6 +714,11 @@
     def lde(self, log_blowup):
         return self._unary(self.ctx.L.wf_mat_lde, log_blowup)
 
+    def interpolate_lde(self, log_blowup):
+        p, l = vp(), vp()
+        self.ctx.check(self.ctx.L.wf_mat_interpolate_lde(self.ctx.h, self.h, log_blowup, C.byref(p), C.byref(l)))
+        return Mat(self.ctx, p), Mat(self.ctx, l)
+
     def interpolate_with_offset(self, offset):
         return self._unary(self.ctx.L.wf_mat_interpolate_with_offset, offset)
 
diff --git a/winterfell_b200/csrc/capi.cu b/winterfell_b200/csrc/capi.cu
--- a/winterfell_b200/csrc/capi.cu
+++ b/winterfell_b200/csrc/capi.cu
@@ -322,6 +322,80 @@
     return launch_pass(ctx, NTT_CONTIG, p, polys.nseg(), k1 - k0);
 }
 
+static int log2_exact(size_t n, u32* out) {
+    if (n == 0 || (n & (n - 1))) return -1;
+    u32 l = 0;
+    while (((size_t)1 << l) < n) l++;
+    *out = l;
+    return 0;
+}
+
+int interpolate_and_extend(wf_ctx* ctx, const wf_mat* evals, u32 log_b, wf_mat** polys_out, wf_mat** lde_out, const char* mark) {
+    u32 log_n;
+    if (log2_exact(evals->m.rows, &log_n) || log_n < 1) return wf_fail(ctx, WF_ERR_INVALID, "rows must be a power of two >= 2");
+    if (log_b > 7 || log_n + log_b > 32) return wf_fail(ctx, WF_ERR_INVALID, "bad blowup");
+    const bool fused = log_n == 2 * NTT_MAX_LOGS && evals->m.W == 8 && seg_width_for(evals->m.cols) == 8 && log_b <= 3;
+    if (!fused) {
+        CKI(wf_mat_interpolate(ctx, evals, polys_out));
+        if (mark) wf_mark(ctx, mark);
+        const int r = wf_mat_lde(ctx, *polys_out, log_b, lde_out);
+        if (r != WF_OK) { wf_mat_free(ctx, *polys_out); *polys_out = nullptr; }
+        return r;
+    }
+    const u32 lr = NTT_MAX_LOGS, nseg = (u32)evals->m.nseg(), b = 1u << log_b;
+    wf_mat *polys = nullptr, *lde = nullptr;
+    void* tp = nullptr;
+    int rc = wf_mat_alloc_w(ctx, evals->m.rows, evals->m.cols, evals->m.W, &polys);
+    if (rc == WF_OK) rc = wf_dev_alloc(ctx, evals->m.words() * 8, &tp);
+    if (rc == WF_OK) rc = wf_mat_alloc(ctx, evals->m.rows << log_b, evals->m.cols, &lde);
+    NttPassParams p;
+    if (rc == WF_OK) {
+        SegMatrix tmp = evals->m;
+        tmp.base = (u64*)tp;
+        pass_defaults(p, evals->m, tmp);
+        p.logS = (int)lr; p.logR = lr; p.logC = lr; p.inverse = 1;
+        p.has_post = 1; p.logM = log_n; p.a_mul = 1; p.b_mul = 0; p.cconst = gl_inv(((u64)1 << log_n) % GL_P);
+        rc = launch_pass(ctx, NTT_STRIDED, p, nseg, 1);
+    }
+    if (rc == WF_OK && mark) wf_mark(ctx, mark);
+    TraceExtendParams t{};
+    LdeTables tabs;
+    if (rc == WF_OK) rc = get_round_tw(ctx, lr, &t.sub_tw);
+    if (rc == WF_OK) rc = get_lde_tables(ctx, log_n, log_b, lr, &tabs);
+    if (rc == WF_OK) {
+        t.logM = log_n + log_b;
+        t.tw_split = t.logM / 2;
+        rc = get_pow_table(ctx, t.logM, t.tw_split, &t.tw_lo);
+    }
+    if (rc == WF_OK) rc = get_pow_table(ctx, t.logM - t.tw_split, t.logM - t.tw_split, &t.tw_hi);
+    if (rc == WF_OK) {
+        t.in = (const u64*)tp; t.polys = polys->m.base; t.lde = lde->m.base;
+        t.in_seg_stride = evals->m.seg_stride; t.polys_seg_stride = polys->m.seg_stride; t.lde_seg_stride = lde->m.seg_stride;
+        t.log_b = log_b; t.pre_tab = tabs.pre; t.ctab = tabs.pow7;
+        wf_use_device(ctx);
+        const cudaError_t e = trace_extend_launch(t, nseg, ctx->st);
+        ctx->launches++;
+        if (e != cudaSuccess) rc = wf_fail(ctx, WF_ERR_CUDA, "trace_extend_kernel: %s", cudaGetErrorString(e));
+    }
+    wf_dev_free(ctx, tp);
+    if (rc == WF_OK) {
+        pass_defaults(p, polys->m, lde->m);
+        p.in = lde->m.base;
+        p.in_seg_stride = lde->m.seg_stride;
+        p.logS = (int)lr; p.logR = lr; p.logC = lr;
+        p.y_in_out = 1; p.out_row_mul = b; p.out_row_add = 1;
+        rc = launch_pass(ctx, NTT_CONTIG, p, nseg, b);
+    }
+    if (rc != WF_OK) {
+        wf_mat_free(ctx, polys);
+        wf_mat_free(ctx, lde);
+        return rc;
+    }
+    *polys_out = polys;
+    *lde_out = lde;
+    return WF_OK;
+}
+
 template <int K>
 __device__ __forceinline__ void field_shift_store(u64 a, u64* out, size_t n, size_t i, int slot) { out[(4 + slot) * n + i] = gl_mul_2exp<K>(a); }
 __global__ void field_ops_kernel(const u64* a, const u64* b, size_t n, u64* out) {
@@ -603,14 +677,6 @@
     return WF_OK;
 }
 
-static int log2_exact(size_t n, u32* out) {
-    if (n == 0 || (n & (n - 1))) return -1;
-    u32 l = 0;
-    while (((size_t)1 << l) < n) l++;
-    *out = l;
-    return 0;
-}
-
 static int mat_transform(wf_ctx* ctx, const wf_mat* in, int inverse, wf_mat** out) {
     if (!ctx || !in || !out) return wf_fail(ctx, WF_ERR_INVALID, "bad arguments");
     u32 log_n;
@@ -644,6 +710,11 @@
     if (r != WF_OK) { wf_mat_free(ctx, o); return r; }
     *lde = o;
     return WF_OK;
+}
+
+int wf_mat_interpolate_lde(wf_ctx* ctx, const wf_mat* evals, uint32_t log_blowup, wf_mat** polys, wf_mat** lde) {
+    if (!ctx || !evals || !polys || !lde) return wf_fail(ctx, WF_ERR_INVALID, "bad arguments");
+    return interpolate_and_extend(ctx, evals, log_blowup, polys, lde, nullptr);
 }
 
 int wf_mat_lde_into(wf_ctx* ctx, const wf_mat* polys, uint32_t log_blowup, wf_mat* lde) {
diff --git a/winterfell_b200/csrc/internal.hpp b/winterfell_b200/csrc/internal.hpp
--- a/winterfell_b200/csrc/internal.hpp
+++ b/winterfell_b200/csrc/internal.hpp
@@ -138,6 +138,7 @@
 extern "C" int wf_trace_lde_cosetwise(wf_ctx* ctx, const uint64_t* const* cols, const uint64_t* d_cols, uint32_t ncols, size_t nrows, int mont,
                            uint32_t log_blowup, wf_mat** polys_out, wf_mat** lde_out, bool coset_major,
                            const std::function<int(u32)>* after_coset);
+int interpolate_and_extend(wf_ctx* ctx, const wf_mat* evals, u32 log_b, wf_mat** polys_out, wf_mat** lde_out, const char* mark);
 extern "C" int wf_mat_lde_cosets(wf_ctx* ctx, const wf_mat* polys, uint32_t log_blowup, uint32_t k0, uint32_t k1, wf_mat* lde);
 extern "C" int wf_mat_lde_from_coset(wf_ctx* ctx, const wf_mat* polys, uint32_t log_blowup, uint32_t k0, wf_mat* lde);
 struct PublicCoin;
diff --git a/winterfell_b200/csrc/ntt.cuh b/winterfell_b200/csrc/ntt.cuh
--- a/winterfell_b200/csrc/ntt.cuh
+++ b/winterfell_b200/csrc/ntt.cuh
@@ -51,3 +51,17 @@
 cudaError_t ntt2_launch_pass(int mode, const NttPassParams& p, u32 n_segments, u32 n_batch, cudaStream_t st);
 size_t ntt2_tw_entries(int logS);
 cudaError_t ntt2_build_tw(int logS, u64* d_out, cudaStream_t st);
+
+struct TraceExtendParams {
+    const u64* in;
+    u64* polys;
+    u64* lde;
+    size_t in_seg_stride, polys_seg_stride, lde_seg_stride;
+    u32 log_b;
+    const u64* sub_tw;
+    const u64* pre_tab;
+    const u64* ctab;
+    const u64 *tw_hi, *tw_lo;
+    u32 tw_split, logM;
+};
+cudaError_t trace_extend_launch(const TraceExtendParams& p, u32 n_segments, cudaStream_t st);
diff --git a/winterfell_b200/csrc/ntt2.cu b/winterfell_b200/csrc/ntt2.cu
--- a/winterfell_b200/csrc/ntt2.cu
+++ b/winterfell_b200/csrc/ntt2.cu
@@ -1,178 +1,4 @@
-#include "minidft.cuh"
-#include "ntt.cuh"
-
-#ifndef NTT2_THREADS
-#define NTT2_THREADS 256
-#endif
-#ifndef NTT2_MINB
-#define NTT2_MINB 2
-#endif
-#define NTT2_TILE_ELEMS 8192
-
-template <int LOGS>
-struct Plan {
-    static constexpr int rounds = LOGS >= 9 ? 3 : 2;
-    static constexpr int r0 = (LOGS == 8) ? 4 : 3;
-    static constexpr int r1 = (LOGS == 11 || LOGS == 8 || LOGS == 7) ? 4 : 3;
-    static constexpr int r2 = LOGS >= 9 ? LOGS - r0 - r1 : 0;
-    static_assert(LOGS >= 6 && LOGS <= 11, "plan covers 2^6 .. 2^11");
-    static_assert(r0 + r1 + r2 == LOGS && (rounds == 2 || (r2 == 3 || r2 == 4)), "radices must add up");
-    static constexpr int lanes = LOGS == 11 ? 4 : 8;
-    static constexpr int tw0_entries = 1 << LOGS;
-    static constexpr int tw1_entries = rounds == 3 ? (1 << (LOGS - r0)) : 0;
-    static constexpr int tw_entries = tw0_entries + tw1_entries;
-};
-template <int LOGS> __host__ __device__ constexpr int plan_radix(int k) { return k == 0 ? Plan<LOGS>::r0 : (k == 1 ? Plan<LOGS>::r1 : Plan<LOGS>::r2); }
-template <int LOGS> __host__ __device__ constexpr int plan_stage(int k) { return k == 0 ? 0 : (k == 1 ? Plan<LOGS>::r0 : Plan<LOGS>::r0 + Plan<LOGS>::r1); }
-
-template <int LK>
-__host__ __device__ constexpr u32 swz_const(u32 r) {
-    u32 x = r >> LK, h = 0;
-    while (x) { h ^= x & ((1u << LK) - 1); x >>= LK; }
-    return h;
-}
-template <int LK>
-__host__ __device__ constexpr u32 swz_lo(u32 Q) { return swz_const<LK>(Q) ^ (Q & ((1u << LK) - 1)); }
-template <int LK>
-__host__ __device__ constexpr u32 swz_hi(u32 Q) { return Q & ~((1u << LK) - 1); }
-__host__ __device__ constexpr u32 brev_const(u32 v, int bits) {
-    u32 r = 0;
-    for (int i = 0; i < bits; i++) r |= ((v >> i) & 1u) << (bits - 1 - i);
-    return r;
-}
-template <int LOGS, int LK, u32 STEP, u32 N, u32 IT = 0, class F>
-__device__ __forceinline__ void for_brev_rows(F&& f) {
-    if constexpr (IT < N) {
-        constexpr u32 c = brev_const(IT * STEP, LOGS);
-        f(IT, swz_lo<LK>(c), swz_hi<LK>(c));
-        for_brev_rows<LOGS, LK, STEP, N, IT + 1>(f);
-    }
-}
-template <int LK>
-__device__ __forceinline__ u32 swz_hash(u32 r) {
-    if (LK == 1) return __popc(r >> 1) & 1;
-    u32 x = r >> 2;
-    x ^= x >> 4;
-    x ^= x >> 8;
-    x ^= x >> 2;
-    return x & 3;
-}
-template <int LK>
-__device__ __forceinline__ u32 prow(u32 r) { return r ^ swz_hash<LK>(r); }
-
-__device__ __forceinline__ void bulk_init(u64* mbar, int tid) {
-    if (tid == 0) {
-        u32 mb = (u32)__cvta_generic_to_shared(mbar);
-        asm volatile("mbarrier.init.shared::cta.b64 [%0], 1;" ::"r"(mb));
-        asm volatile("fence.mbarrier_init.release.cluster;" ::: "memory");
-    }
-}
-__device__ __forceinline__ void bulk_expect(u64* mbar, u32 bytes) {
-    u32 mb = (u32)__cvta_generic_to_shared(mbar);
-    asm volatile("mbarrier.arrive.expect_tx.shared::cta.b64 _, [%0], %1;" ::"r"(mb), "r"(bytes) : "memory");
-}
-__device__ __forceinline__ void bulk_copy(void* smem_dst, const void* gsrc, u32 bytes, u64* mbar) {
-    u32 mb = (u32)__cvta_generic_to_shared(mbar), dst = (u32)__cvta_generic_to_shared(smem_dst);
-    asm volatile("cp.async.bulk.shared::cluster.global.mbarrier::complete_tx::bytes [%0], [%1], %2, [%3];" ::"r"(dst), "l"(gsrc), "r"(bytes),
-                 "r"(mb)
-                 : "memory");
-}
-__device__ __forceinline__ void bulk_wait(u64* mbar) {
-    u32 mb = (u32)__cvta_generic_to_shared(mbar), done = 0;
-    while (!done)
-        asm volatile("{\n\t.reg .pred p;\n\tmbarrier.try_wait.parity.shared::cta.b64 p, [%1], 0;\n\tselp.u32 %0, 1, 0, p;\n\t}" : "=r"(done) : "r"(mb) : "memory");
-}
-
-__device__ __forceinline__ void cp_async16(void* smem_dst, const void* gsrc, bool ok) {
-    const u32 dst = (u32)__cvta_generic_to_shared(smem_dst);
-    asm volatile("cp.async.cg.shared.global [%0], [%1], 16, %2;" ::"r"(dst), "l"(gsrc), "r"(ok ? 16 : 0) : "memory");
-}
-__device__ __forceinline__ void cp_async8(void* smem_dst, const void* gsrc, bool ok) {
-    const u32 dst = (u32)__cvta_generic_to_shared(smem_dst);
-    asm volatile("cp.async.ca.shared.global [%0], [%1], 8, %2;" ::"r"(dst), "l"(gsrc), "r"(ok ? 8 : 0) : "memory");
-}
-__device__ __forceinline__ void cp_async_commit() { asm volatile("cp.async.commit_group;" ::: "memory"); }
-__device__ __forceinline__ void cp_async_wait_all() { asm volatile("cp.async.wait_group 0;" ::: "memory"); }
-
-template <int LOGS, int K>
-__device__ __forceinline__ void tile_round(u64* __restrict__ s, const u64* __restrict__ tw, const u64* __restrict__ pre, int tid) {
-    constexpr int LANES = Plan<LOGS>::lanes, LK = LANES == 8 ? 1 : 2;
-    constexpr int R = plan_radix<LOGS>(K), ST = plan_stage<LOGS>(K);
-    constexpr int LOGSPAN = LOGS - ST - R;
-    constexpr u32 SPAN = 1u << LOGSPAN;
-    constexpr bool LAST = LOGSPAN == 0;
-    constexpr u32 TASKS = (1u << LOGS) * LANES / 16;
-    if (R == 4) {
-#pragma unroll 1
-        for (u32 task = tid; task < TASKS; task += NTT2_THREADS) {
-            const u32 lane = task % LANES, bf = task / LANES;
-            const u32 lo = bf & (SPAN - 1), base = ((bf >> LOGSPAN) << (LOGSPAN + 4)) + lo;
-            const u32 bh = base ^ swz_hash<LK>(base);
-            u64* pr[1 << LK];
-#pragma unroll
-            for (int v = 0; v < (1 << LK); v++) pr[v] = s + ((bh ^ v) * LANES + lane);
-            u64 x[16];
-#pragma unroll
-            for (int q = 0; q < 16; q++) x[q] = pr[swz_lo<LK>((u32)q << LOGSPAN)][swz_hi<LK>((u32)q << LOGSPAN) * LANES];
-            if (K == 0 && pre) {
-#pragma unroll
-                for (int q = 0; q < 16; q++) x[q] = gl_mul(x[q], __ldg(pre + base + ((u32)q << LOGSPAN)));
-            }
-            mini_dft<4>(x);
-            if (!LAST) {
-                const ulonglong2* t2 = reinterpret_cast<const ulonglong2*>(tw + (size_t)lo * 16);
-#pragma unroll
-                for (int h = 0; h < 8; h++) {
-                    const ulonglong2 w = t2[h];
-                    if (h > 0) x[2 * h] = gl_mul(x[2 * h], w.x);
-                    x[2 * h + 1] = gl_mul(x[2 * h + 1], w.y);
-                }
-            }
-#pragma unroll
-            for (int q = 0; q < 16; q++) pr[swz_lo<LK>((u32)q << LOGSPAN)][swz_hi<LK>((u32)q << LOGSPAN) * LANES] = x[q];
-        }
-    } else {
-        constexpr int LP = LANES / 2;
-#pragma unroll 1
-        for (u32 task = tid; task < TASKS; task += NTT2_THREADS) {
-            const u32 lp = task % LP, bf = task / LP;
-            const u32 lo = bf & (SPAN - 1), base = ((bf >> LOGSPAN) << (LOGSPAN + 3)) + lo;
-            const u32 bh = base ^ swz_hash<LK>(base);
-            ulonglong2* pr[1 << LK];
-#pragma unroll
-            for (int v = 0; v < (1 << LK); v++) pr[v] = reinterpret_cast<ulonglong2*>(s + ((bh ^ v) * LANES + 2 * lp));
-            u64 xa[8], xb[8];
-#pragma unroll
-            for (int q = 0; q < 8; q++) {
-                const ulonglong2 v = pr[swz_lo<LK>((u32)q << LOGSPAN)][swz_hi<LK>((u32)q << LOGSPAN) * (LANES / 2)];
-                xa[q] = v.x;
-                xb[q] = v.y;
-            }
-            if (K == 0 && pre) {
-#pragma unroll
-                for (int q = 0; q < 8; q++) {
-                    const u64 f = __ldg(pre + base + ((u32)q << LOGSPAN));
-                    xa[q] = gl_mul(xa[q], f);
-                    xb[q] = gl_mul(xb[q], f);
-                }
-            }
-            mini_dft<3>(xa);
-            mini_dft<3>(xb);
-            if (!LAST) {
-                const ulonglong2* t2 = reinterpret_cast<const ulonglong2*>(tw + (size_t)lo * 8);
-#pragma unroll
-                for (int h = 0; h < 4; h++) {
-                    const ulonglong2 w = t2[h];
-                    if (h > 0) { xa[2 * h] = gl_mul(xa[2 * h], w.x); xb[2 * h] = gl_mul(xb[2 * h], w.x); }
-                    xa[2 * h + 1] = gl_mul(xa[2 * h + 1], w.y);
-                    xb[2 * h + 1] = gl_mul(xb[2 * h + 1], w.y);
-                }
-            }
-#pragma unroll
-            for (int q = 0; q < 8; q++) pr[swz_lo<LK>((u32)q << LOGSPAN)][swz_hi<LK>((u32)q << LOGSPAN) * (LANES / 2)] = make_ulonglong2(xa[q], xb[q]);
-        }
-    }
-}
+#include "ntt2.cuh"
 
 template <int MODE, int LOGS>
 __global__ void __launch_bounds__(NTT2_THREADS, NTT2_MINB) ntt2_pass_kernel(const NttPassParams p) {
diff --git a/winterfell_b200/csrc/ntt2.cuh b/winterfell_b200/csrc/ntt2.cuh
--- /dev/null
+++ b/winterfell_b200/csrc/ntt2.cuh
@@ -0,0 +1,180 @@
+#pragma once
+#include "minidft.cuh"
+#include "ntt.cuh"
+
+#ifndef NTT2_THREADS
+#define NTT2_THREADS 256
+#endif
+#ifndef NTT2_MINB
+#define NTT2_MINB 2
+#endif
+#define NTT2_TILE_ELEMS 8192
+
+template <int LOGS>
+struct Plan {
+    static constexpr int rounds = LOGS >= 9 ? 3 : 2;
+    static constexpr int r0 = (LOGS == 8) ? 4 : 3;
+    static constexpr int r1 = (LOGS == 11 || LOGS == 8 || LOGS == 7) ? 4 : 3;
+    static constexpr int r2 = LOGS >= 9 ? LOGS - r0 - r1 : 0;
+    static_assert(LOGS >= 6 && LOGS <= 11, "plan covers 2^6 .. 2^11");
+    static_assert(r0 + r1 + r2 == LOGS && (rounds == 2 || (r2 == 3 || r2 == 4)), "radices must add up");
+    static constexpr int lanes = LOGS == 11 ? 4 : 8;
+    static constexpr int tw0_entries = 1 << LOGS;
+    static constexpr int tw1_entries = rounds == 3 ? (1 << (LOGS - r0)) : 0;
+    static constexpr int tw_entries = tw0_entries + tw1_entries;
+};
+template <int LOGS> __host__ __device__ constexpr int plan_radix(int k) { return k == 0 ? Plan<LOGS>::r0 : (k == 1 ? Plan<LOGS>::r1 : Plan<LOGS>::r2); }
+template <int LOGS> __host__ __device__ constexpr int plan_stage(int k) { return k == 0 ? 0 : (k == 1 ? Plan<LOGS>::r0 : Plan<LOGS>::r0 + Plan<LOGS>::r1); }
+
+template <int LK>
+__host__ __device__ constexpr u32 swz_const(u32 r) {
+    u32 x = r >> LK, h = 0;
+    while (x) { h ^= x & ((1u << LK) - 1); x >>= LK; }
+    return h;
+}
+template <int LK>
+__host__ __device__ constexpr u32 swz_lo(u32 Q) { return swz_const<LK>(Q) ^ (Q & ((1u << LK) - 1)); }
+template <int LK>
+__host__ __device__ constexpr u32 swz_hi(u32 Q) { return Q & ~((1u << LK) - 1); }
+__host__ __device__ constexpr u32 brev_const(u32 v, int bits) {
+    u32 r = 0;
+    for (int i = 0; i < bits; i++) r |= ((v >> i) & 1u) << (bits - 1 - i);
+    return r;
+}
+template <int LOGS, int LK, u32 STEP, u32 N, u32 IT = 0, class F>
+__device__ __forceinline__ void for_brev_rows(F&& f) {
+    if constexpr (IT < N) {
+        constexpr u32 c = brev_const(IT * STEP, LOGS);
+        f(IT, swz_lo<LK>(c), swz_hi<LK>(c));
+        for_brev_rows<LOGS, LK, STEP, N, IT + 1>(f);
+    }
+}
+template <int LK>
+__device__ __forceinline__ u32 swz_hash(u32 r) {
+    if (LK == 1) return __popc(r >> 1) & 1;
+    u32 x = r >> 2;
+    x ^= x >> 4;
+    x ^= x >> 8;
+    x ^= x >> 2;
+    return x & 3;
+}
+template <int LK>
+__device__ __forceinline__ u32 prow(u32 r) { return r ^ swz_hash<LK>(r); }
+
+__device__ __forceinline__ void bulk_init(u64* mbar, int tid) {
+    if (tid == 0) {
+        u32 mb = (u32)__cvta_generic_to_shared(mbar);
+        asm volatile("mbarrier.init.shared::cta.b64 [%0], 1;" ::"r"(mb));
+        asm volatile("fence.mbarrier_init.release.cluster;" ::: "memory");
+    }
+}
+__device__ __forceinline__ void bulk_expect(u64* mbar, u32 bytes) {
+    u32 mb = (u32)__cvta_generic_to_shared(mbar);
+    asm volatile("mbarrier.arrive.expect_tx.shared::cta.b64 _, [%0], %1;" ::"r"(mb), "r"(bytes) : "memory");
+}
+__device__ __forceinline__ void bulk_copy(void* smem_dst, const void* gsrc, u32 bytes, u64* mbar) {
+    u32 mb = (u32)__cvta_generic_to_shared(mbar), dst = (u32)__cvta_generic_to_shared(smem_dst);
+    asm volatile("cp.async.bulk.shared::cluster.global.mbarrier::complete_tx::bytes [%0], [%1], %2, [%3];" ::"r"(dst), "l"(gsrc), "r"(bytes),
+                 "r"(mb)
+                 : "memory");
+}
+__device__ __forceinline__ void bulk_wait(u64* mbar) {
+    u32 mb = (u32)__cvta_generic_to_shared(mbar), done = 0;
+    while (!done)
+        asm volatile("{\n\t.reg .pred p;\n\tmbarrier.try_wait.parity.shared::cta.b64 p, [%1], 0;\n\tselp.u32 %0, 1, 0, p;\n\t}" : "=r"(done) : "r"(mb) : "memory");
+}
+
+__device__ __forceinline__ void cp_async16(void* smem_dst, const void* gsrc, bool ok) {
+    const u32 dst = (u32)__cvta_generic_to_shared(smem_dst);
+    asm volatile("cp.async.cg.shared.global [%0], [%1], 16, %2;" ::"r"(dst), "l"(gsrc), "r"(ok ? 16 : 0) : "memory");
+}
+__device__ __forceinline__ void cp_async8(void* smem_dst, const void* gsrc, bool ok) {
+    const u32 dst = (u32)__cvta_generic_to_shared(smem_dst);
+    asm volatile("cp.async.ca.shared.global [%0], [%1], 8, %2;" ::"r"(dst), "l"(gsrc), "r"(ok ? 8 : 0) : "memory");
+}
+__device__ __forceinline__ void cp_async_commit() { asm volatile("cp.async.commit_group;" ::: "memory"); }
+__device__ __forceinline__ void cp_async_wait_all() { asm volatile("cp.async.wait_group 0;" ::: "memory"); }
+
+template <int LOGS, int K>
+__device__ __forceinline__ void tile_round(u64* __restrict__ s, const u64* __restrict__ tw, const u64* __restrict__ pre, int tid) {
+    constexpr int LANES = Plan<LOGS>::lanes, LK = LANES == 8 ? 1 : 2;
+    constexpr int R = plan_radix<LOGS>(K), ST = plan_stage<LOGS>(K);
+    constexpr int LOGSPAN = LOGS - ST - R;
+    constexpr u32 SPAN = 1u << LOGSPAN;
+    constexpr bool LAST = LOGSPAN == 0;
+    constexpr u32 TASKS = (1u << LOGS) * LANES / 16;
+    if (R == 4) {
+#pragma unroll 1
+        for (u32 task = tid; task < TASKS; task += NTT2_THREADS) {
+            const u32 lane = task % LANES, bf = task / LANES;
+            const u32 lo = bf & (SPAN - 1), base = ((bf >> LOGSPAN) << (LOGSPAN + 4)) + lo;
+            const u32 bh = base ^ swz_hash<LK>(base);
+            u64* pr[1 << LK];
+#pragma unroll
+            for (int v = 0; v < (1 << LK); v++) pr[v] = s + ((bh ^ v) * LANES + lane);
+            u64 x[16];
+#pragma unroll
+            for (int q = 0; q < 16; q++) x[q] = pr[swz_lo<LK>((u32)q << LOGSPAN)][swz_hi<LK>((u32)q << LOGSPAN) * LANES];
+            if (K == 0 && pre) {
+#pragma unroll
+                for (int q = 0; q < 16; q++) x[q] = gl_mul(x[q], __ldg(pre + base + ((u32)q << LOGSPAN)));
+            }
+#ifndef NTT2_NO_ROUNDS
+            mini_dft<4>(x);
+            if (!LAST) {
+                const ulonglong2* t2 = reinterpret_cast<const ulonglong2*>(tw + (size_t)lo * 16);
+#pragma unroll
+                for (int h = 0; h < 8; h++) {
+                    const ulonglong2 w = t2[h];
+                    if (h > 0) x[2 * h] = gl_mul(x[2 * h], w.x);
+                    x[2 * h + 1] = gl_mul(x[2 * h + 1], w.y);
+                }
+            }
+#endif
+#pragma unroll
+            for (int q = 0; q < 16; q++) pr[swz_lo<LK>((u32)q << LOGSPAN)][swz_hi<LK>((u32)q << LOGSPAN) * LANES] = x[q];
+        }
+    } else {
+        constexpr int LP = LANES / 2;
+#pragma unroll 1
+        for (u32 task = tid; task < TASKS; task += NTT2_THREADS) {
+            const u32 lp = task % LP, bf = task / LP;
+            const u32 lo = bf & (SPAN - 1), base = ((bf >> LOGSPAN) << (LOGSPAN + 3)) + lo;
+            const u32 bh = base ^ swz_hash<LK>(base);
+            ulonglong2* pr[1 << LK];
+#pragma unroll
+            for (int v = 0; v < (1 << LK); v++) pr[v] = reinterpret_cast<ulonglong2*>(s + ((bh ^ v) * LANES + 2 * lp));
+            u64 xa[8], xb[8];
+#pragma unroll
+            for (int q = 0; q < 8; q++) {
+                const ulonglong2 v = pr[swz_lo<LK>((u32)q << LOGSPAN)][swz_hi<LK>((u32)q << LOGSPAN) * (LANES / 2)];
+                xa[q] = v.x;
+                xb[q] = v.y;
+            }
+            if (K == 0 && pre) {
+#pragma unroll
+                for (int q = 0; q < 8; q++) {
+                    const u64 f = __ldg(pre + base + ((u32)q << LOGSPAN));
+                    xa[q] = gl_mul(xa[q], f);
+                    xb[q] = gl_mul(xb[q], f);
+                }
+            }
+#ifndef NTT2_NO_ROUNDS
+            mini_dft<3>(xa);
+            mini_dft<3>(xb);
+            if (!LAST) {
+                const ulonglong2* t2 = reinterpret_cast<const ulonglong2*>(tw + (size_t)lo * 8);
+#pragma unroll
+                for (int h = 0; h < 4; h++) {
+                    const ulonglong2 w = t2[h];
+                    if (h > 0) { xa[2 * h] = gl_mul(xa[2 * h], w.x); xb[2 * h] = gl_mul(xb[2 * h], w.x); }
+                    xa[2 * h + 1] = gl_mul(xa[2 * h + 1], w.y);
+                    xb[2 * h + 1] = gl_mul(xb[2 * h + 1], w.y);
+                }
+            }
+#endif
+#pragma unroll
+            for (int q = 0; q < 8; q++) pr[swz_lo<LK>((u32)q << LOGSPAN)][swz_hi<LK>((u32)q << LOGSPAN) * (LANES / 2)] = make_ulonglong2(xa[q], xb[q]);
+        }
+    }
+}
diff --git a/winterfell_b200/csrc/ntt_fused.cu b/winterfell_b200/csrc/ntt_fused.cu
--- /dev/null
+++ b/winterfell_b200/csrc/ntt_fused.cu
@@ -0,0 +1,155 @@
+#include "ntt2.cuh"
+
+namespace {
+constexpr int TX_LOGS = 11, TX_LANES = 4, TX_LK = 2, TX_LP = TX_LANES / 2;
+constexpr u32 TX_S = 1u << TX_LOGS;
+constexpr u32 TX_ROWS_PER_IT = NTT2_THREADS / TX_LP;
+static_assert(Plan<TX_LOGS>::lanes == TX_LANES && Plan<TX_LOGS>::r0 == 3, "round 0 of the 2^11-point plan is radix-8 on lane pairs");
+constexpr int TX_R0_SPAN_LOG = TX_LOGS - Plan<TX_LOGS>::r0;
+
+__device__ __forceinline__ void st_global_128(u64* p, u64 a, u64 b) {
+    asm volatile("st.global.v2.u64 [%0], {%1, %2};" ::"l"(p), "l"(a), "l"(b));
+}
+}
+
+__global__ void __launch_bounds__(NTT2_THREADS, NTT2_MINB) trace_extend_kernel(const TraceExtendParams p) {
+    extern __shared__ __align__(16) u64 smem[];
+    constexpr int LOGS = TX_LOGS, LANES = TX_LANES, LK = TX_LK, LP = TX_LP;
+    constexpr u32 S = TX_S, ROWS_PER_IT = TX_ROWS_PER_IT;
+    const int tid = threadIdx.x;
+    u64* s = smem;
+    u64* rtw = s + (size_t)S * LANES;
+    u64* ctw = rtw + Plan<LOGS>::tw_entries;
+    u64* mbar = ctw + S;
+    const u32 j1 = blockIdx.x >> 1, q0 = (blockIdx.x & 1) * LANES, g = blockIdx.y;
+    const u32 nb = 1u << p.log_b;
+    const u32 lp = tid % LP, l0 = 2 * lp;
+
+    {
+        const u64* a0 = p.in + (size_t)g * p.in_seg_stride + ((size_t)j1 << LOGS) * 8 + q0 + l0;
+#pragma unroll 4
+        for (u32 i = tid / LP; i < S; i += ROWS_PER_IT) cp_async16(s + prow<LK>(i) * LANES + l0, a0 + (size_t)i * 8, true);
+        cp_async_commit();
+    }
+    bulk_init(mbar, tid);
+    __syncthreads();
+    if (tid == 0) {
+        bulk_expect(mbar, Plan<LOGS>::tw_entries * 8);
+        bulk_copy(rtw, p.sub_tw, Plan<LOGS>::tw_entries * 8, mbar);
+    }
+    const u32 M = 1u << p.logM, lo_mask = (1u << p.tw_split) - 1, m = j1;
+    auto wpow = [&](u64 e64) {
+        const u32 e = (u32)(e64 & (M - 1));
+        return gl_mul(p.tw_hi[e >> p.tw_split], p.tw_lo[e & lo_mask]);
+    };
+    {
+        const u64 step = wpow((u64)NTT2_THREADS * nb * m);
+        u64 x = gl_mul(p.ctab[m], wpow((u64)tid * nb * m));
+        for (u32 j = tid; j < S; j += NTT2_THREADS) {
+            ctw[j] = x;
+            x = gl_mul(x, step);
+        }
+    }
+    if (tid == 0) mbar[1] = wpow(m);
+    cp_async_wait_all();
+    bulk_wait(mbar);
+    __syncthreads();
+
+    tile_round<LOGS, 0>(s, rtw, nullptr, tid);
+    __syncthreads();
+    tile_round<LOGS, 1>(s, rtw + Plan<LOGS>::tw0_entries, nullptr, tid);
+    __syncthreads();
+    tile_round<LOGS, 2>(s, nullptr, nullptr, tid);
+    __syncthreads();
+
+    ulonglong2 cf[2][8];
+    {
+        u32 t = tid;
+        asm volatile("" : "+r"(t));
+        u64* po = p.polys + (size_t)g * p.polys_seg_stride + (size_t)j1 * 8 + q0 + 2 * (t % LP);
+#pragma unroll
+        for (int it = 0; it < 2; it++) {
+            const u32 bf = t / LP + (u32)it * (NTT2_THREADS / LP);
+#pragma unroll
+            for (int q = 0; q < 8; q++) {
+                const u32 i = bf + ((u32)q << TX_R0_SPAN_LOG);
+                const u32 r = __brev((S - i) & (S - 1)) >> (32 - LOGS);
+                cf[it][q] = *reinterpret_cast<const ulonglong2*>(s + prow<LK>(r) * LANES + 2 * (t % LP));
+                *reinterpret_cast<ulonglong2*>(po + ((size_t)i << LOGS) * 8) = cf[it][q];
+            }
+        }
+    }
+    __syncthreads();
+
+    const u64 jstride = (u64)nb * 8, ostep = (u64)ROWS_PER_IT * jstride;
+    for (u32 k = 0; k < nb; k++) {
+        u32 t = tid;
+        asm volatile("" : "+r"(t));
+        if (k) {
+            const u64 kstep = mbar[1];
+            for (u32 j = tid; j < S; j += NTT2_THREADS) ctw[j] = gl_mul(ctw[j], kstep);
+        }
+        const u64* pre = p.pre_tab + ((size_t)k << LOGS);
+#pragma unroll
+        for (int it = 0; it < 2; it++) {
+            const u32 bf = t / LP + (u32)it * (NTT2_THREADS / LP);
+            const u32 bh = bf ^ swz_hash<LK>(bf);
+            ulonglong2* pr[1 << LK];
+#pragma unroll
+            for (int v = 0; v < (1 << LK); v++) pr[v] = reinterpret_cast<ulonglong2*>(s + ((bh ^ v) * LANES + 2 * (t % LP)));
+            u64 xa[8], xb[8];
+#pragma unroll
+            for (int q = 0; q < 8; q++) {
+                const u64 f = __ldg(pre + bf + ((u32)q << TX_R0_SPAN_LOG));
+                xa[q] = gl_mul(cf[it][q].x, f);
+                xb[q] = gl_mul(cf[it][q].y, f);
+            }
+#ifndef NTT2_NO_ROUNDS
+            mini_dft<3>(xa);
+            mini_dft<3>(xb);
+            const ulonglong2* t2 = reinterpret_cast<const ulonglong2*>(rtw + (size_t)bf * 8);
+#pragma unroll
+            for (int h = 0; h < 4; h++) {
+                const ulonglong2 w = t2[h];
+                if (h > 0) { xa[2 * h] = gl_mul(xa[2 * h], w.x); xb[2 * h] = gl_mul(xb[2 * h], w.x); }
+                xa[2 * h + 1] = gl_mul(xa[2 * h + 1], w.y);
+                xb[2 * h + 1] = gl_mul(xb[2 * h + 1], w.y);
+            }
+#endif
+#pragma unroll
+            for (int q = 0; q < 8; q++)
+                pr[swz_lo<LK>((u32)q << TX_R0_SPAN_LOG)][swz_hi<LK>((u32)q << TX_R0_SPAN_LOG) * (LANES / 2)] = make_ulonglong2(xa[q], xb[q]);
+        }
+        __syncthreads();
+        tile_round<LOGS, 1>(s, rtw + Plan<LOGS>::tw0_entries, nullptr, tid);
+        __syncthreads();
+        tile_round<LOGS, 2>(s, nullptr, nullptr, tid);
+        __syncthreads();
+        {
+            u32 t = tid;
+            asm volatile("" : "+r"(t));
+            const u32 j0 = t / LP, r0 = __brev(j0) >> (32 - LOGS), rh = r0 ^ swz_hash<LK>(r0), w0 = q0 + 2 * (t % LP);
+            const ulonglong2* pr[1 << LK];
+#pragma unroll
+            for (int v = 0; v < (1 << LK); v++) pr[v] = reinterpret_cast<const ulonglong2*>(s + ((rh ^ v) * LANES + w0 - q0));
+            const u64* cj = ctw + j0;
+            u64* oj = p.lde + (size_t)g * p.lde_seg_stride + ((((size_t)m << LOGS) + j0) * nb + k) * 8 + w0;
+            for_brev_rows<LOGS, LK, ROWS_PER_IT, S / ROWS_PER_IT>([&](u32 it, u32 lo, u32 hi) {
+                ulonglong2 v = pr[lo][hi * (LANES / 2)];
+                const u64 f = cj[it * ROWS_PER_IT];
+                v.x = gl_mul(v.x, f);
+                v.y = gl_mul(v.y, f);
+                st_global_128(oj + it * ostep, v.x, v.y);
+            });
+        }
+        __syncthreads();
+    }
+}
+
+cudaError_t trace_extend_launch(const TraceExtendParams& p, u32 n_segments, cudaStream_t st) {
+    const size_t smem = ((size_t)TX_S * TX_LANES + Plan<TX_LOGS>::tw_entries + TX_S + 2) * 8;
+    cudaError_t e = cudaFuncSetAttribute(trace_extend_kernel, cudaFuncAttributeMaxDynamicSharedMemorySize, (int)smem);
+    if (e != cudaSuccess) return e;
+    trace_extend_kernel<<<dim3(2 * TX_S, n_segments), NTT2_THREADS, smem, st>>>(p);
+    return cudaGetLastError();
+}
diff --git a/winterfell_b200/csrc/prover.cu b/winterfell_b200/csrc/prover.cu
--- a/winterfell_b200/csrc/prover.cu
+++ b/winterfell_b200/csrc/prover.cu
@@ -1203,10 +1203,14 @@
     if (d_trace) {
         CKI(wf_mat_from_device_columns(ctx, d_trace, c, n, &trace));
         wf_mark(ctx, "trace_upload_layout");
-        CKI(wf_mat_interpolate(ctx, trace, &polys));
-        if (!aux_build && !validate) scope.drop(trace);
-        wf_mark(ctx, "trace_interpolate");
-        CKI(wf_mat_lde(ctx, polys, log_b, &lde));
+        if (!aux_build && !validate) {
+            CKI(interpolate_and_extend(ctx, trace, log_b, &polys, &lde, "trace_interpolate"));
+            scope.drop(trace);
+        } else {
+            CKI(wf_mat_interpolate(ctx, trace, &polys));
+            wf_mark(ctx, "trace_interpolate");
+            CKI(wf_mat_lde(ctx, polys, log_b, &lde));
+        }
     } else {
         CKI(wf_trace_lde_from_host(ctx, trace_cols, c, n, mont, log_b, &polys, &lde));
     }
```

Result: faster. 77.11, median of 6 (-3.1%).
